# Korinin38/raytracing-hw

Hardware: AMD Instinct MI355X
Metric: Mrays/sec + frame time, Sponza 1920x1080x256spp at 1/2/4/8 MI355X (higher is better)
Workload: dtype f32

## Files before the change

### raytracing-hw_amd/csrc/rt_device.hip

```cpp
#include <hip/hip_runtime.h>
#include <hipcub/hipcub.hpp>

#include <algorithm>
#include <chrono>
#include <cstdio>
#include <cstdlib>
#include <cstring>
#include <mutex>
#include <string>
#include <thread>
#include <vector>

#include "rt_path.h"
#include "rt_wavefront.h"
#include <type_traits>
#include "rt_mega.h"
#include "rt_quant_lut.h"
#include "rt_scene.h"
#include "rt_bvh_layout.h"
#include "rt_launch_plan.h"
#include "rt_select.h"
#include "rt_frame_plan.h"
#include "rt_gbuffer.h"
#include "rt_denoise.h"

using rtd::Counters;
using rtd::DevScene;
using rtd::ShardGeom;
using rtd::shard_row;

#ifndef RT_MEGA_WPE
#define RT_MEGA_WPE 5
#endif
constexpr int kMegaWpe = RT_MEGA_WPE;
#ifndef RT_SPEC_WPE
#define RT_SPEC_WPE 4
#endif
constexpr int kMegaWpeSpec = RT_SPEC_WPE;
#ifndef RT_SHADE_MIN
#define RT_SHADE_MIN 48
#endif
#ifndef RT_SPEC_SHADE_MIN
#define RT_SPEC_SHADE_MIN 44
#endif
constexpr int kSpecShadeMin = RT_SPEC_SHADE_MIN;
constexpr int kShadeMin = RT_SHADE_MIN;
#ifndef RT_PACK_TRAV
#define RT_PACK_TRAV 1
#endif
constexpr bool kPackTrav = RT_PACK_TRAV != 0;
#ifndef RT_INV_RECOMPUTE
#define RT_INV_RECOMPUTE 1
#endif
constexpr bool kInvRecompute = RT_INV_RECOMPUTE != 0;
#ifndef RT_COOP_LEAVES
#define RT_COOP_LEAVES 8
#endif
constexpr int kCoopLeavesPlain = RT_COOP_LEAVES;
#ifndef RT_SPEC_COOP_LEAVES
#define RT_SPEC_COOP_LEAVES 12
#endif
constexpr int kCoopLeavesSpec = RT_SPEC_COOP_LEAVES;
#ifndef RT_SPEC_MASK_LOAD
#define RT_SPEC_MASK_LOAD 1
#endif
constexpr bool kSpecMaskLoad = RT_SPEC_MASK_LOAD != 0;
#ifndef RT_PLAIN_FAR_DIST2
#define RT_PLAIN_FAR_DIST2 RT_FAR_DIST2
#endif
#ifndef RT_SPEC_FAR_DIST2
#define RT_SPEC_FAR_DIST2 0
#endif
constexpr bool kPlainFarDist2 = RT_PLAIN_FAR_DIST2 != 0, kSpecFarDist2 = RT_SPEC_FAR_DIST2 != 0;
#ifndef RT_COOP_ROUND_MIN
#define RT_COOP_ROUND_MIN 8
#endif
constexpr int kCoopRoundMinPlain = RT_COOP_ROUND_MIN;
#ifndef RT_ORDER_SPP
#define RT_ORDER_SPP 1
#endif
#ifndef RT_ORDER_RADIUS
#define RT_ORDER_RADIUS 4
#endif
constexpr int kOrderSpp = RT_ORDER_SPP;
constexpr int kOrderRadius = RT_ORDER_RADIUS;
using rtp::kClaimStride;
constexpr int kWfRefill = 8;
constexpr unsigned kWfChunk = 64;
constexpr double kWfCompactBelow = 0.75;

struct rt_device_blob {
    std::vector<uint8_t> bytes;
    size_t o_tri, o_attr, o_tan, o_node, o_light, o_lnode, o_mf, o_mt, o_nt, o_ti, o_tx, o_lut;
};

struct rt_device_scene {
    int device = -1;
    void *buf = nullptr;
    DevScene ds{};
    unsigned long long *counters = nullptr;
    unsigned long long *queue = nullptr;
    int cu_count = 0;
    void *wf_buf = nullptr;
    long long wf_cap = 0;
    int wf_D = 0;
    rtd::WfState wf{};
    float4 *wf_queue[2] = {nullptr, nullptr};
    float4 *wf_hits = nullptr;
    unsigned *wf_count = nullptr;
    unsigned *wf_fetch = nullptr;
    unsigned *wf_host_count = nullptr;
    float *fast_part = nullptr;
    size_t fast_part_bytes = 0;
    void *order_buf = nullptr;
    size_t order_bytes = 0;
    struct Frame {
        hipStream_t stream = nullptr, cp_stream = nullptr;
        void *buf[2] = {nullptr, nullptr};
        size_t bytes[2] = {0, 0};
        hipEvent_t copied[2] = {nullptr, nullptr};
        hipEvent_t finished = nullptr;
        hipEvent_t last = nullptr;
        void *root_buf = nullptr;
        size_t root_bytes = 0;
    } fr;
};

#define HIP_TRY(expr)                                                                          \
    do {                                                                                       \
        hipError_t _e = (expr);                                                                \
        if (_e != hipSuccess)                                                                  \
            return rt_fail(RT_ERR_DEVICE, std::string(#expr) + ": " + hipGetErrorString(_e)); \
    } while (0)

namespace {

struct DeviceGuard {
    int prev = -1;
    bool ok = false;
    explicit DeviceGuard(int dev) {
        if (hipGetDevice(&prev) != hipSuccess) prev = -1;
        ok = hipSetDevice(dev) == hipSuccess;
    }
    ~DeviceGuard() {
        if (prev >= 0) (void)hipSetDevice(prev);
    }
};

struct EventSet {
    std::vector<hipEvent_t> ev;
    hipError_t make(hipEvent_t &e) {
        hipError_t r = hipEventCreate(&e);
        if (r == hipSuccess) ev.push_back(e);
        return r;
    }
    ~EventSet() {
        for (hipEvent_t e : ev) (void)hipEventDestroy(e);
    }
};

hipError_t grow(void **p, size_t *cap, size_t need) {
    if (*p && *cap >= need) return hipSuccess;
    if (*p) (void)hipFree(*p);
    *p = nullptr;
    *cap = 0;
    hipError_t e = hipMalloc(p, need ? need : 256);
    if (e == hipSuccess) *cap = need;
    return e;
}

}

__constant__ uint32_t k_quant_thr[256];
__global__ void __launch_bounds__(256) rt_finish_kernel(const float *sum, long long n, float normalizer,
                                                         uint8_t *rgb) {
    __shared__ float thr[256];
    thr[threadIdx.x] = __uint_as_float(k_quant_thr[threadIdx.x]);
    __syncthreads();
    for (long long i = (long long)blockIdx.x * blockDim.x + threadIdx.x; i < n; i += (long long)gridDim.x * blockDim.x) {
        float x = sum[i];
        x *= normalizer;
        const float num = x * (x * 2.51f + 0.03f);
        const float den = x * (x * 2.43f + 0.59f) + 0.14f;
        const float v = rtv::smax(rtv::smin(num / den, 1.f), 0.f);
        int q = 0;
        if (!isnan(v)) {
            int lo = 0;
#pragma unroll
            for (int step = 128; step > 0; step >>= 1)
                if (lo + step <= 255 && thr[lo + step] <= v) lo += step;
            q = lo;
        }
        rgb[i] = (uint8_t)q;
    }
}

__global__ void __launch_bounds__(256) rt_finish_counts_kernel(const float *sum, const int32_t *counts, long long n,
                                                                uint8_t *rgb) {
    __shared__ float thr[256];
    thr[threadIdx.x] = __uint_as_float(k_quant_thr[threadIdx.x]);
    __syncthreads();
    for (long long i = (long long)blockIdx.x * blockDim.x + threadIdx.x; i < n; i += (long long)gridDim.x * blockDim.x) {
        const int32_t c = counts[i / 3];
        float x = sum[i];
        x *= rtsel::count_normalizer(c);
        const float num = x * (x * 2.51f + 0.03f);
        const float den = x * (x * 2.43f + 0.59f) + 0.14f;
        const float v = rtv::smax(rtv::smin(num / den, 1.f), 0.f);
        int q = 0;
        if (c > 0 && !isnan(v)) {
            int lo = 0;
#pragma unroll
            for (int step = 128; step > 0; step >>= 1)
                if (lo + step <= 255 && thr[lo + step] <= v) lo += step;
            q = lo;
        }
        rgb[i] = (uint8_t)q;
    }
}

#ifdef RT_MEGA_PROF
#include "rt_mega_prof.h"
#endif
template <bool COUNT, bool FAST = false, bool LSPLIT = false, bool SPEC = false, bool CHAIN = false>
__global__ void __launch_bounds__(256) __attribute__((amdgpu_waves_per_eu(SPEC ? kMegaWpeSpec : kMegaWpe, 8)))
rt_mega_kernel(DevScene sc_in, ShardGeom g, rtd::WfState st, int spp, float *out, unsigned long long *counters,
               unsigned long long *queue, const int *order, unsigned *cost, int cs, int mode) {
    constexpr bool kSpec = SPEC && !COUNT && !FAST && !LSPLIT;
    constexpr bool kChain = CHAIN && !COUNT && !FAST && !LSPLIT;
    constexpr bool kFastChain = CHAIN && FAST && !COUNT && !LSPLIT && !SPEC;
    const int park_below = kFastChain ? 0 : rtp::mode_park_below(mode), resume_pct = kFastChain ? 0 : rtp::mode_resume_pct(mode);
    const uint4 *resume = kSpec && resume_pct > 0 ? (const uint4 *)queue[rtd::kQueueParkList] : nullptr;
    const long long n_items = kFastChain ? st.n * (long long)mode
                              : FAST     ? g.n_pixels * (long long)((spp + cs - 1) / cs)
                                         : (kChain || (kSpec && resume)) ? st.n : g.n_pixels;
    const int lane = threadIdx.x & 63;
    __shared__ float lut[256];
    for (int k = threadIdx.x; k < 256; k += blockDim.x) lut[k] = sc_in.lut[k];
    __syncthreads();
    DevScene sc = sc_in;
    sc.lut = lut;
    Counters cnt{0, 0, 0, 0, 0, 0, 0};
    constexpr int kK = kSpec ? rtd::kLdsStackSpec : rtd::kLdsStack;
    uint2 spill[rtd::kStack - kK];
    rtd::LdsStackT<kK> S{spill};
    const rtd::GlobalNodes nodes{sc.node};
    const rtd::NodeRec root = rtd::load_node(sc.node, 0);
    std::conditional_t<kSpec, rtd::MegaLane, rtd::MegaLaneU> L;
    L.pix = -1;
    L.state = rtd::M_IDLE;
    L.T.phase = rtd::TP_POP;
    L.T.sp = 0;
#if defined(RT_DEBUG_CHECKS)
    if (rt_debug_poison) {
        L.T.phase = 0x7ffffffd;
        L.T.sp = 0x3ffffff;
    }
#endif
    L.wbase = (uint32_t)__builtin_amdgcn_readfirstlane((int)threadIdx.x) & ~63u;
    bool exhausted = false;
    bool tail = false, wave_room = false;
#ifdef RT_MEGA_PROF
    unsigned long long pf[7] = {0, 0, 0, 0, 0, 0, 0};
    if (threadIdx.x < 8) rt_prof_lds[threadIdx.x] = 0;
    if (threadIdx.x < 16) rtd::spec_prof_lds[threadIdx.x] = 0;
    if ((threadIdx.x & 63) == 0) rtd::spec_wave_t0_lds[threadIdx.x >> 6] = wall_clock64();
    __syncthreads();
    long long tp = clock64();
    const unsigned long long wt0 = wall_clock64();
    TbAcc tbk;
#endif
    rtd::SpecClaim claim{queue + rtd::kQueueResume, 0, n_items, resume, 0, false,
                         resume ? (const int *)queue[rtd::kQueueResumeMap] : nullptr};
    bool park = false;
    if constexpr (kSpec) {
        if (resume) {
            const long long waves = (long long)gridDim.x * (blockDim.x >> 6);
            const long long dealt = (n_items * resume_pct + 99) / 100;
            const int per = (int)std::min<long long>(64, std::max<long long>(1, (dealt + waves - 1) / waves));
            const long long p = (rtd::mega_slot() >> 6) * per + lane;
            bool xk = false;
            rtd::Rng xs{0u, 0u, 0.f};
            if (lane < per && p < n_items) {
                const rtd::Parked q = rtd::parked_item(resume, claim.ridx, p);
                if (q.pix != rtd::kNoPark) {
                    rtd::mega_resume(L, sc, g, q, root);
                    xk = true;
                    xs = q.x;
                }
            }
            exhausted = true;
            claim.base = waves * per;
            claim.keep = per;
            claim.open = claim.base < n_items;
            if (lane == 0) rtd::spec_hint_take();
            rtd::spec_convert(L, sc, g, rtd::SpecView{(uint4 *)st.mid, st.lanes, rtd::mega_slot() - lane}, lane, xk, xs);
            tail = true;
#ifdef RT_MEGA_PROF
            if (lane == 0) RT_SPEC_STAT(7, 1);
#endif
        }
    }
#if defined(RT_DEBUG_CHECKS)
    unsigned long long dbg_iter = 0;
#endif
    for (;;) {
#if defined(RT_DEBUG_CHECKS)
        if (++dbg_iter > (1ull << 22)) {
            const unsigned long long w = (unsigned long long)__popcll(__ballot(L.state == rtd::M_TRAV)) |
                                         (unsigned long long)__popcll(__ballot(L.state == rtd::M_READY)) << 8 |
                                         (unsigned long long)__popcll(__ballot(L.state == rtd::M_DONE)) << 16 |
                                         (unsigned long long)__popcll(__ballot(L.state == rtd::M_DONE_NEW)) << 24 |
                                         (unsigned long long)__popcll(__ballot(L.state == rtd::M_IDLE)) << 32 |
                                         (unsigned long long)tail << 40 | (unsigned long long)park << 41 |
                                         (unsigned long long)exhausted << 42 | (unsigned long long)wave_room << 43;
            RT_CHECK(false, 15, w, (void)0);
            if constexpr (kSpec) {
                const rtd::SpecView V{(uint4 *)st.mid, st.lanes, rtd::mega_slot() - lane};
                const uint4 a = *V.w(0, lane), b = *V.w(1, lane), c = *V.w(2, lane), d = *V.w(3, lane), j = *V.w(4, lane);
                if (atomicAdd(&rt_debug_prints, 1u) < 64u)
                    printf("[stuck] blk %d lane %d state %d pix %d s %d | job tag %u | rec pix %u f %u n %u e %u meta %u tab %08x%08x\n",
                           (int)blockIdx.x, lane, L.state, L.pix, rtd::lane_ctr(L).s, j.x, a.x, a.y, a.z, a.w, b.w, d.w, c.w);
            }
            break;
        }
#endif
        if (!kSpec && !COUNT && !FAST && park) {
            if (L.state == rtd::M_IDLE && L.pix >= 0) {
                rtd::park_pixel((uint4 *)queue[rtd::kQueueParkList], rtd::mega_slot_of(L), L.pix, rtd::lane_ctr(L).s, rtd::lane_rng(L),
                                rtd::lane_sum(L));
                L.pix = -1;
            }
        }
        if (!exhausted) {
            const bool need = L.pix < 0 && (kClaimStride == 1 || lane % kClaimStride == 0);
            const unsigned long long m = __ballot(need);
            if (m) {
                const int leader = __ffsll((unsigned long long)m) - 1;
                const unsigned cm = (unsigned)__popcll(m);
                const int below = (int)__builtin_amdgcn_mbcnt_hi((uint32_t)(m >> 32), __builtin_amdgcn_mbcnt_lo((uint32_t)m, 0u));
                unsigned long long base = 0;
                if (need && below == 0) base = atomicAdd(queue + rtd::kQueueRender, (unsigned long long)cm);
                base = __shfl(base, leader, 64);
                if (need) {
                    const long long p = (long long)base + below;
                    if (p < n_items) {
                        if constexpr (kFastChain)
                            rtd::mega_assign_fast_chain<COUNT>(L, sc, g, p, st.n, order, cs, spp, root, cnt, rtd::chain_of(queue));
                        else if (FAST) rtd::mega_assign_fast<COUNT>(L, sc, g, p, cs, spp, root, cnt);
                        else if constexpr (kChain)
                            rtd::mega_assign_chain<COUNT>(L, sc, g, order ? order[p] : (int)p, root, cnt, rtd::chain_of(queue), spp);
                        else rtd::mega_assign<COUNT>(L, sc, g, order ? order[p] : (int)p, root, cnt);
                    }
                }
                if ((long long)base + cm >= n_items) exhausted = true;
            }
        }
        if constexpr (kSpec) {
            if (exhausted && !tail) {
                if (lane == 0) rtd::spec_hint_take();
                if constexpr (kChain)
                    rtd::spec_convert_chain(L, sc, g, rtd::SpecView{(uint4 *)st.mid, st.lanes, rtd::mega_slot() - lane}, lane,
                                            rtd::chain_of(queue));
                else
                    rtd::spec_convert(L, sc, g, rtd::SpecView{(uint4 *)st.mid, st.lanes, rtd::mega_slot() - lane}, lane);
                tail = true;
                wave_room = false;
#ifdef RT_MEGA_PROF
                if (lane == 0) RT_SPEC_STAT(7, 1);
#endif
            }
            if (tail) {
                wave_room |= rtd::spec_hint_take();
                if (__any(L.state == rtd::M_DONE_NEW) || (wave_room && __any(L.state == rtd::M_IDLE))) {
#ifdef RT_MEGA_PROF
                    const long long c0 = clock64();
                    tbk.c[5] += 1;
#endif
                    wave_room = rtd::spec_manage<kChain>(rtd::SpecLanes{L}, sc, g,
                                                 rtd::SpecView{(uint4 *)st.mid, st.lanes, rtd::mega_slot() - lane}, spp,
                                                 out, root, claim);
#ifdef RT_MEGA_PROF
                    if (lane == 0) {
                        RT_SPEC_STAT(0, 1);
                        RT_SPEC_STAT(1, clock64() - c0);
                    }
#endif
                }
                if (!__any(L.state != rtd::M_IDLE)) break;
            } else if (!__any(L.pix >= 0)) {
                break;
            }
        } else if constexpr (kFastChain) {
            if (!__any(L.pix >= 0)) {
                if (exhausted) break;
                continue;
            }
        } else if (!__any(L.pix >= 0)) {
            break;
        }
        if (!kSpec && park_below > 0 && exhausted && !park) park = rtp::park_rule(__popcll(__ballot(L.pix >= 0)), park_below);
        const int nr = __popcll(__ballot(L.state == rtd::M_READY || (LSPLIT && L.state == rtd::M_LREADY)));
        const int nt = __popcll(__ballot(L.state == rtd::M_TRAV || (LSPLIT && L.state == rtd::M_LTRAV)));
        const bool shade_now = nr > 0 && (nr >= (kSpec ? kSpecShadeMin : kShadeMin) || nt == 0);
        if constexpr (kSpec) {
            if (shade_now) __builtin_amdgcn_s_setprio(0);
            else __builtin_amdgcn_s_setprio(1);
        }
#ifdef RT_MEGA_PROF
        {
            const long long t1 = clock64();
            pf[2] += (unsigned long long)(t1 - tp);
            tp = t1;
            pf[shade_now ? 3 : 4] += 1;
            pf[shade_now ? 5 : 6] += (unsigned long long)(shade_now ? nr : nt);
            tbk.at(wt0);
            if (shade_now) {
                tbk.c[3] += 1;
                tbk.c[4] += (unsigned long long)nr;
            }
        }
#endif
        if (!LSPLIT && !shade_now) {
            int kt = nt;
            int leaf_defer = 0;
            do {
                if (rtd::trav_step_coop<COUNT, kSpec ? kCoopLeavesSpec : kCoopLeavesPlain, kSpec && kSpecMaskLoad,
                                        kSpec ? rtd::kLeafDefer : (COUNT ? 0 : rtd::kLeafDeferPlain),
                                        kSpec ? kSpecFarDist2 : kPlainFarDist2>(
                        sc, L.r, L.T, S, nodes, cnt, L.state == rtd::M_TRAV, kSpec ? st.round_min : kCoopRoundMinPlain,
                        rtd::NoHook{}, &leaf_defer))
                    L.state = rtd::M_READY;
                const unsigned long long rb = __ballot(L.state == rtd::M_READY), tb = __ballot(L.state == rtd::M_TRAV);
                kt = __popcll(tb);
                if (kt == 0 || __popcll(rb) >= (kSpec ? kSpecShadeMin : kShadeMin)) break;
#ifdef RT_MEGA_PROF
                pf[4] += 1;
                pf[6] += (unsigned long long)kt;
                tbk.c[0] += 1;
                tbk.c[1] += (unsigned long long)kt;
                tbk.c[2] += (unsigned long long)__popcll(__ballot(L.state != rtd::M_IDLE));
#endif
            } while (true);
        } else if (kPackTrav && !LSPLIT && !kSpec && !FAST) {
            RT_CHECK((unsigned)L.T.phase < 4u && (unsigned)L.state < 8u && (unsigned)L.T.sp <= (unsigned)rtd::kStack, 14,
                     (unsigned)L.T.phase | (unsigned long long)(unsigned)L.state << 32, (void)0);
            uint32_t pk = ((uint32_t)L.T.phase & 3u) | ((uint32_t)L.state & 7u) << 2 | ((uint32_t)L.T.sp & 127u) << 5;
            asm volatile("" : "+v"(pk));
            if (L.state == rtd::M_READY) {
                L.T.phase = 0;
                L.T.sp = 0;
                rtd::mega_shade<COUNT, FAST, kChain>(L, sc, g, st, spp, out, cost, root, S, cnt, kSpec && tail, park, queue);
            } else {
                L.T.phase = (int)(pk & 3u);
                L.state = (int)((pk >> 2) & 7u);
                L.T.sp = (int)(pk >> 5);
            }
        } else {
            rtd::mega_iterate<COUNT, decltype(S), decltype(nodes), FAST, LSPLIT, kChain>(L, shade_now, sc, g, st, spp, out,
                                                                                       cost, root, S, nodes, cnt,
                                                                                       kSpec && tail, false, queue);
            if (kInvRecompute && shade_now) L.r.inv = rtv::divv(rtd::V3{1.f, 1.f, 1.f}, L.r.d);
        }
        if (kPackTrav && kInvRecompute && !LSPLIT && !kSpec && !FAST && shade_now)
            L.r.inv = rtv::divv(rtd::V3{1.f, 1.f, 1.f}, L.r.d);

#ifdef RT_MEGA_PROF
        {
            const long long t1 = clock64();
            pf[shade_now ? 0 : 1] += (unsigned long long)(t1 - tp);
            tp = t1;
        }
#endif
    }
#ifdef RT_MEGA_PROF
    tbk.flush(tbk.b);
    if (lane == 0) {
        for (int k = 0; k < 7; ++k) atomicAdd(&g_mega_prof[k], pf[k]);
        atomicAdd(&g_mega_prof[7], 1ull);
        const unsigned wi = atomicAdd(&g_wave_n, 1u);
        if (wi < (unsigned)kProfWaves) {
            g_wave_t[2 * wi] = wt0;
            g_wave_t[2 * wi + 1] = wall_clock64();
        }
    }
    __syncthreads();
    if (threadIdx.x < 8) atomicAdd(&g_mega_seg[threadIdx.x], rt_prof_lds[threadIdx.x]);
    if (threadIdx.x < 16) atomicAdd(&rtd::g_spec_prof[threadIdx.x], rtd::spec_prof_lds[threadIdx.x]);
#endif
    rtd::counters_flush<COUNT>(cnt, counters);
}

__global__ void __launch_bounds__(256) rt_fast_reduce_kernel(const float *__restrict__ part, float *__restrict__ out,
                                                             long long n3, int chunks) {
    const long long i = (long long)blockIdx.x * blockDim.x + threadIdx.x;
    if (i >= n3) return;
    float s = 0.f;
    for (int c = 0; c < chunks; ++c) s += part[(long long)c * n3 + i];
    out[i] = s;
}

struct FastPartials {
    const float *part;
    long long n_list, i;
    RT_HD float operator()(int k, int ch) const { return part[3 * ((long long)k * n_list + i) + ch]; }
};
__global__ void __launch_bounds__(256) rt_fast_fold_chain_kernel(uint4 *chain, const int *items, long long n_list, int units,
                                                                  int c, int target, const float *__restrict__ part,
                                                                  float *sums) {
    const long long i = (long long)blockIdx.x * blockDim.x + threadIdx.x;
    if (i >= n_list) return;
    const long long p = items ? (long long)items[i] : i;
    rtd::FastRec q = rtd::fast_rec(chain, p);
    const int own = rtfu::units_of(q.r.next, target, c);
    if (own < 1 || own > units) return;
    rtfu::fold(q.r, target, c, FastPartials{part, n_list, i});
    rtd::fast_rec_store(chain, p, q.r);
    float s[3];
    rtfu::reported(q.r, c, s);
    sums[3 * p + 0] = s[0];
    sums[3 * p + 1] = s[1];
    sums[3 * p + 2] = s[2];
}

__global__ void __launch_bounds__(256) rt_order_iota_kernel(int *ids, long long n) {
    const long long i = (long long)blockIdx.x * blockDim.x + threadIdx.x;
    if (i < n) ids[i] = (int)i;
}

__global__ void __launch_bounds__(256) rt_order_box_kernel(const unsigned *in, unsigned *out, long long n, int width,
                                                           int r, int dir) {
    const long long p = (long long)blockIdx.x * blockDim.x + threadIdx.x;
    if (p >= n) return;
    const long long rows = n / width, k = p / width, i = p % width;
    unsigned s = 0;
    for (int d = -r; d <= r; ++d) {
        const long long kk = dir ? k + d : k, ii = dir ? i : i + d;
        if (kk >= 0 && kk < rows && ii >= 0 && ii < width) s += in[kk * width + ii];
    }
    out[p] = s;
}

__global__ void __launch_bounds__(256) rt_order_spread_kernel(const int *sorted, int *order, long long n,
                                                              long long groups, long long per) {
    const long long q = (long long)blockIdx.x * blockDim.x + threadIdx.x;
    if (q >= n) return;
    const long long m = n < groups * per ? n : groups * per;
    long long r = q;
    if (q < m) {
        const long long gi = q / per, j = q % per, a = m / per, b = m % per;
        r = j * a + (j < b ? j : b) + gi;
    }
    order[q] = sorted[r];
}

__global__ void __launch_bounds__(256) rt_park_keys_kernel(const uint4 *park, long long n, int spp, const unsigned *est,
                                                           unsigned *keys, int *ids) {
    const long long i = (long long)blockIdx.x * blockDim.x + threadIdx.x;
    if (i >= n) return;
    const rtd::Parked q = rtd::parked(park, i);
    unsigned long long k = 0;
    if (q.pix != rtd::kNoPark) k = (unsigned long long)(spp - (int)q.s) * ((unsigned long long)est[q.pix] + 1ull);
    keys[i] = k > 0xffffffffull ? 0xffffffffu : (unsigned)k;
    ids[i] = (int)i;
}
__global__ void rt_set_u64_kernel(unsigned long long *dst, unsigned long long v) { *dst = v; }

__global__ void __launch_bounds__(256) wf_init_kernel(DevScene sc, ShardGeom g, rtd::WfState st, long long n,
                                                       float4 *qout, unsigned *cout) {
    for (long long base = (long long)blockIdx.x * blockDim.x; base < n; base += (long long)gridDim.x * blockDim.x) {
        const long long i = base + threadIdx.x;
        const bool valid = i < n;
        if (valid) rtd::store_qray(sc, qout, (unsigned)i, (int)i, rtd::wf_init_slot(sc, g, st, i));
        rtd::queue_slot(valid, cout);
    }
}

template <bool COUNT>
__global__ void __launch_bounds__(256) wf_extend_kernel(DevScene sc, const float4 *qin, const unsigned *count,
                                                         unsigned npos, float4 *hits, unsigned *fetch,
                                                         unsigned *next_count, unsigned long long *counters) {
    const unsigned n = npos ? npos : *count;
    if (blockIdx.x == 0 && threadIdx.x == 0) {
        atomicAdd(&counters[7], (unsigned long long)n);
        *next_count = 0;
    }
    Counters cnt{0, 0, 0, 0, 0, 0, 0};
    uint2 spill[rtd::kStack - rtd::kLdsStackWf];
    rtd::LdsStackT<rtd::kLdsStackWf> S{spill};
    const int lane = threadIdx.x & 63;
    const rtd::GlobalNodes nodes{sc.node};
    const rtd::NodeRec root = rtd::load_node(sc.node, 0);
    unsigned q = 0, lo = 0, hi = 0;
    bool busy = false, exhausted = false;
    rtd::Ray r;
    rtd::TravState T;
    for (;;) {
        const unsigned long long m = __ballot(!busy);
        const unsigned idle = (unsigned)__popcll(m);
        if (!exhausted && (idle >= (unsigned)kWfRefill || idle == 64)) {
            const unsigned rank = (unsigned)__popcll(m & ((1ull << lane) - 1ull));
            unsigned got = 0, mine = 0xffffffffu;
            while (got < idle) {
                if (lo >= hi) {
                    unsigned b = 0;
                    if (lane == 0) b = atomicAdd(fetch, kWfChunk);
                    b = __shfl(b, 0, 64);
                    if (b >= n) {
                        exhausted = true;
                        break;
                    }
                    lo = b;
                    hi = b + kWfChunk < n ? b + kWfChunk : n;
                }
                const unsigned k = hi - lo < idle - got ? hi - lo : idle - got;
                if (!busy && rank >= got && rank < got + k) mine = lo + (rank - got);
                lo += k;
                got += k;
            }
            if (mine != 0xffffffffu) {
                q = mine;
                uint32_t bits;
                int slot;
                r = rtd::load_qray_trav(qin, q, bits, slot);
                if (slot >= 0) {
                    busy = rtd::trav_start<COUNT>(bits, root.a, root.b, T, cnt);
                    if (!busy) rtd::store_hit(hits, q, T.best);
                }
            }
        }
        if (busy && rtd::trav_step<COUNT>(sc, r, T, S, nodes, cnt)) {
            rtd::store_hit(hits, q, T.best);
            busy = false;
        }
        if (exhausted && !__any(busy)) break;
    }
    rtd::counters_flush<COUNT>(cnt, counters);
}

constexpr int kMatLds = 64;
struct ShadeLds {
    float lut[512];
    float mf[kMatLds * 12];
    int mt[kMatLds * 4];
    double nt[kMatLds * 16];
};

template <bool COUNT, bool MAT_LDS>
__global__ void __launch_bounds__(256) wf_shade_kernel(DevScene sc_in, ShardGeom g, rtd::WfState st, int spp,
                                                        const float4 *qin, const unsigned *cin, unsigned npos,
                                                        const float4 *hits, float4 *qout, unsigned *cout,
                                                        int dense_out, unsigned *fetch, float *out,
                                                        unsigned long long *counters) {
    __shared__ ShadeLds L;
    for (int k = threadIdx.x; k < 512; k += blockDim.x) L.lut[k] = sc_in.lut[k];
    if (MAT_LDS) {
        for (int k = threadIdx.x; k < sc_in.n_meshes * 12; k += blockDim.x) L.mf[k] = sc_in.mesh_f[k];
        for (int k = threadIdx.x; k < sc_in.n_meshes * 4; k += blockDim.x) L.mt[k] = sc_in.mesh_tex[k];
        for (int k = threadIdx.x; k < sc_in.n_meshes * 16; k += blockDim.x) L.nt[k] = sc_in.mesh_nt[k];
    }
    __syncthreads();
    DevScene sc = sc_in;
    sc.lut = L.lut;
    if (MAT_LDS) {
        sc.mesh_f = L.mf;
        sc.mesh_tex = L.mt;
        sc.mesh_nt = L.nt;
    }
    const unsigned n = npos ? npos : *cin;
    if (blockIdx.x == 0 && threadIdx.x == 0) *fetch = 0;
    Counters cnt{0, 0, 0, 0, 0, 0, 0};
    for (unsigned base = blockIdx.x * blockDim.x; base < n; base += gridDim.x * blockDim.x) {
        const unsigned q = base + threadIdx.x;
        int slot = -1;
        bool next = false;
        rtd::Ray r;
        if (q < n) {
            r = rtd::load_qray(qin, q, slot);
            if (slot >= 0) {
                const rtd::Hit h = rtd::load_hit(hits, q);
                next = rtd::wf_shade_slot<COUNT>(sc, g, st, spp, slot, r, h, out, cnt);
            }
        }
        const unsigned p = rtd::queue_slot(next, cout);
        if (dense_out) {
            if (next) rtd::store_qray(sc, qout, q, slot, r);
            else if (q < n) rtd::store_qray_inactive(qout, q);
        } else if (next) {
            rtd::store_qray(sc, qout, p, slot, r);
        }
    }
    rtd::counters_flush<COUNT>(cnt, counters);
}

__global__ void __launch_bounds__(256) rt_rays_kernel(DevScene sc, long long n, const float *org, const float *dir,
                                                       float *out_f, long long *out_i) {
    const long long k = (long long)blockIdx.x * blockDim.x + threadIdx.x;
    if (k >= n) return;
    rtd::Ray r = rtd::make_ray(rtv::V3{org[3 * k], org[3 * k + 1], org[3 * k + 2]},
                               rtv::V3{dir[3 * k], dir[3 * k + 1], dir[3 * k + 2]});
    Counters c1{0, 0, 0, 0, 0, 0, 0}, c2{0, 0, 0, 0, 0, 0, 0};
    rtd::Hit h;
    const bool ok = rtd::closest_hit<true>(sc, r, h, c1);
    const float lp = sc.n_lights ? rtd::light_pdf<true>(sc, r.o, r.d, c2) : 0.f;
    out_f[4 * k + 0] = ok ? h.t : 0.f;
    out_f[4 * k + 1] = ok ? h.u : 0.f;
    out_f[4 * k + 2] = ok ? h.v : 0.f;
    out_f[4 * k + 3] = lp;
    out_i[6 * k + 0] = ok;
    out_i[6 * k + 1] = ok ? h.prim : -1;
    out_i[6 * k + 2] = c1.aabb;
    out_i[6 * k + 3] = c1.tri;
    out_i[6 * k + 4] = c2.laabb;
    out_i[6 * k + 5] = c2.ltri;
}

namespace {

template <class T>
size_t append(std::vector<uint8_t> &blob, const std::vector<T> &v, size_t pre = 0) {
    size_t off = rtp::align_up(blob.size()) + pre;
    blob.resize(off + v.size() * sizeof(T));
    if (!v.empty()) std::memcpy(blob.data() + off, v.data(), v.size() * sizeof(T));
    return off;
}

void tile_textures(const std::vector<uint32_t> &info, const std::vector<uint8_t> &texels, std::vector<uint32_t> &info_out,
                   std::vector<uint32_t> &out) {
    const size_t n = info.size() / 4;
    info_out = info;
    out.clear();
    for (size_t t = 0; t < n; ++t) {
        const uint32_t off = info[4 * t], w = info[4 * t + 1], h = info[4 * t + 2];
        const uint32_t tw = (w + 3) / 4, th = (h + 3) / 4;
        const size_t base = out.size();
        info_out[4 * t] = (uint32_t)base;
        out.resize(base + (size_t)tw * th * 16, 0u);
        for (uint32_t y = 0; y < h; ++y)
            for (uint32_t x = 0; x < w; ++x) {
                uint32_t v;
                std::memcpy(&v, &texels[4 * ((size_t)off + (size_t)y * w + x)], 4);
                out[base + ((size_t)(y >> 2) * tw + (x >> 2)) * 16 + (y & 3) * 4 + (x & 3)] = v;
            }
    }
}

int ensure_blob(rt_scene *s) {
    if (s->blob) return RT_OK;
    if (s->bvh_depth + 2 >= (uint32_t)rtd::kStack || s->light_bvh_depth + 2 >= (uint32_t)rtd::kStack)
        return rt_fail(RT_ERR_LIMIT, "BVH deeper than the device traversal stack (" + std::to_string(rtd::kStack) + ")");
    if (s->ray_depth > rtd::kMaxDepth) return rt_fail(RT_ERR_LIMIT, "ray_depth exceeds device limit");
    for (size_t k = 0; k < s->node.size() / 8; ++k) {
        uint32_t a, b;
        std::memcpy(&a, &s->node[8 * k + 6], 4);
        std::memcpy(&b, &s->node[8 * k + 7], 4);
        if (a >= rtd::kFrameMaxA || b >= 1024u)
            return rt_fail(RT_ERR_LIMIT, "scene too large for the device BVH frame packing (2^22 nodes/triangles, 255 per leaf)");
    }
    auto *b = new rt_device_blob();
    std::vector<uint8_t> &blob = b->bytes;
    b->o_tri = append(blob, s->tri);
    b->o_attr = append(blob, s->tri_attr);
    b->o_tan = append(blob, s->tri_tan);
    b->o_node = append(blob, rtd::bfs_nodes(s->node), 32);
    b->o_light = append(blob, s->light);
    b->o_lnode = append(blob, s->light_node);
    b->o_mf = append(blob, s->mesh_f);
    b->o_mt = append(blob, s->mesh_tex);
    b->o_nt = append(blob, s->mesh_nt);
    std::vector<uint32_t> tinfo, tiled;
    tile_textures(s->tex_info, s->texels, tinfo, tiled);
    b->o_ti = append(blob, tinfo);
    b->o_tx = append(blob, tiled);
    std::vector<float> lut(512);
    rtd::fill_decode_lut(lut.data());
    b->o_lut = append(blob, lut);
    blob.resize(rtp::align_up(blob.size()) + 256);
    s->blob = b;
    return RT_OK;
}

void free_device_scene(rt_device_scene *d) {
    if (!d) return;
    DeviceGuard guard(d->device);
    if (guard.ok) {
        for (hipStream_t q : {d->fr.stream, d->fr.cp_stream})
            if (q) (void)hipStreamSynchronize(q);
        for (void *p : {d->buf, (void *)d->counters, (void *)d->queue, d->wf_buf, (void *)d->wf_count,
                        (void *)d->wf_fetch, (void *)d->fast_part, d->order_buf, d->fr.buf[0], d->fr.buf[1], d->fr.root_buf})
            if (p) (void)hipFree(p);
        if (d->wf_host_count) (void)hipHostFree(d->wf_host_count);
        for (hipEvent_t e : {d->fr.copied[0], d->fr.copied[1], d->fr.finished, d->fr.last})
            if (e) (void)hipEventDestroy(e);
        for (hipStream_t q : {d->fr.stream, d->fr.cp_stream})
            if (q) (void)hipStreamDestroy(q);
    }
    delete d;
}

hipError_t ensure_frame_streams(rt_device_scene *d) {
    hipError_t e = hipSuccess;
    if (!d->fr.stream) e = hipStreamCreateWithFlags(&d->fr.stream, hipStreamNonBlocking);
    if (e == hipSuccess && !d->fr.cp_stream) e = hipStreamCreateWithFlags(&d->fr.cp_stream, hipStreamNonBlocking);
    for (hipEvent_t *ev : {&d->fr.copied[0], &d->fr.copied[1], &d->fr.finished, &d->fr.last})
        if (e == hipSuccess && !*ev) e = hipEventCreateWithFlags(ev, hipEventDisableTiming);
    return e;
}

int ensure_device_scene(rt_scene *s, int device) {
    if (device < 0 || device >= kRtMaxDevices) return rt_fail(RT_ERR_DEVICE, "no HIP device " + std::to_string(device));
    if (s->dev[device]) return RT_OK;
    int ndev = 0;
    HIP_TRY(hipGetDeviceCount(&ndev));
    if (device >= ndev) return rt_fail(RT_ERR_DEVICE, "no HIP device " + std::to_string(device));
    int rc = ensure_blob(s);
    if (rc) return rc;
    const rt_device_blob &b = *s->blob;
    DeviceGuard guard(device);
    if (!guard.ok) return rt_fail(RT_ERR_DEVICE, "hipSetDevice(" + std::to_string(device) + ") failed");
    rt_device_scene *d = new rt_device_scene();
    d->device = device;
    hipError_t e = hipMalloc(&d->buf, b.bytes.size());
    if (e == hipSuccess) e = hipMemcpy(d->buf, b.bytes.data(), b.bytes.size(), hipMemcpyHostToDevice);
    if (e == hipSuccess) e = hipMalloc((void **)&d->counters, rtd::kCounterWords * sizeof(unsigned long long));
    if (e == hipSuccess) e = hipMalloc((void **)&d->queue, rtd::kQueueWords * sizeof(unsigned long long));
    hipDeviceProp_t prop;
    if (e == hipSuccess) e = hipGetDeviceProperties(&prop, device);
    if (e != hipSuccess) {
        free_device_scene(d);
        return rt_fail(RT_ERR_DEVICE, std::string("scene upload: ") + hipGetErrorString(e));
    }
    d->cu_count = prop.multiProcessorCount;
    uint8_t *base = (uint8_t *)d->buf;
    DevScene &ds = d->ds;
    ds.tri = (const float4 *)(base + b.o_tri);
    ds.tri_attr = (const float4 *)(base + b.o_attr);
    ds.tri_tan = (const float4 *)(base + b.o_tan);
    ds.node = (const float4 *)(base + b.o_node);
    ds.light = (const float4 *)(base + b.o_light);
    ds.light_node = (const float4 *)(base + b.o_lnode);
    ds.mesh_f = (const float *)(base + b.o_mf);
    ds.mesh_tex = (const int *)(base + b.o_mt);
    ds.mesh_nt = (const double *)(base + b.o_nt);
    ds.tex_info = (const uint4 *)(base + b.o_ti);
    ds.texels = (const uint32_t *)(base + b.o_tx);
    ds.lut = (const float *)(base + b.o_lut);
    ds.n_lights = (int)(s->light.size() / 16);
    ds.n_tris = (int)(s->tri.size() / 12);
    ds.n_nodes = (int)(s->node.size() / 8);
    ds.n_meshes = (int)(s->mesh_f.size() / 12);
    ds.ray_depth = s->ray_depth;
    ds.max_distance = s->max_distance;
    ds.width = s->width;
    ds.height = s->height;
    ds.fwidth = (float)s->width;
    ds.fheight = (float)s->height;
    std::memcpy(ds.cam_pos, s->cam_pos, sizeof ds.cam_pos);
    std::memcpy(ds.cam_axes, s->cam_axes, sizeof ds.cam_axes);
    std::memcpy(ds.tan_fov, s->tan_half_fov, sizeof ds.tan_fov);
    s->dev[device] = d;
    return RT_OK;
}

int ensure_wf(rt_device_scene *d, long long n, int D) {
    if (d->wf_buf && d->wf_cap >= n && d->wf_D == D) return RT_OK;
    if (d->wf_buf) (void)hipFree(d->wf_buf);
    d->wf_buf = nullptr;
    d->wf_cap = 0;
    const long long cap = ((n + 255) / 256) * 256;
    const int planes = 8 + 9 * D + 20
                       + 2 * 4 * rtd::kQRec + 4;
    const size_t bytes = (size_t)cap * 4 * (size_t)planes;
    HIP_TRY(hipMalloc(&d->wf_buf, bytes));
    if (!d->wf_count) HIP_TRY(hipMalloc((void **)&d->wf_count, 16));
    if (!d->wf_fetch) HIP_TRY(hipMalloc((void **)&d->wf_fetch, 16));
    if (!d->wf_host_count) HIP_TRY(hipHostMalloc((void **)&d->wf_host_count, 16, hipHostMallocDefault));
    float *f = (float *)d->wf_buf;
    auto take = [&](long long k) { float *p = f; f += (size_t)cap * k; return p; };
    rtd::WfState &w = d->wf;
    w.n = n;
    w.D = D;
    d->wf_queue[0] = (float4 *)take(4 * rtd::kQRec);
    d->wf_queue[1] = (float4 *)take(4 * rtd::kQRec);
    d->wf_hits = (float4 *)take(4);
    w.st = (float4 *)take(8);
    w.rec_ab = (float4 *)take(8 * D);
    w.rec_c = take(D);
    w.mid = (float4 *)take(20);
    {
        const unsigned long long park = (unsigned long long)(uintptr_t)d->wf_queue[0];
        HIP_TRY(hipMemcpy(d->queue + rtd::kQueueParkList, &park, sizeof park, hipMemcpyHostToDevice));
    }
    d->wf_cap = cap;
    d->wf_D = D;
    return RT_OK;
}

template <class K>
long long resident_blocks(rt_device_scene *d, K kernel) {
    int per_cu = 0;
    if (hipOccupancyMaxActiveBlocksPerMultiprocessor(&per_cu, kernel, 256, 0) != hipSuccess || per_cu < 1) per_cu = 1;
    return (long long)d->cu_count * per_cu;
}
template <class K>
unsigned persistent_blocks(rt_device_scene *d, K kernel, long long work) {
    const long long need = (work + 255) / 256;
    const long long b = std::min<long long>(need, resident_blocks(d, kernel));
    return (unsigned)std::max<long long>(b, 1);
}

struct LaunchTimer {
    bool on = false;
    std::vector<hipEvent_t> ev[2];
    hipError_t mark(int k, hipStream_t s) {
        if (!on) return hipSuccess;
        hipEvent_t e;
        hipError_t r = hipEventCreate(&e);
        if (r != hipSuccess) return r;
        ev[k].push_back(e);
        return hipEventRecord(e, s);
    }
    hipError_t collect(double ms[2], uint64_t n[2]) {
        hipError_t r = hipSuccess;
        for (int k = 0; k < 2; ++k) {
            ms[k] = 0.0;
            n[k] = ev[k].size() / 2;
            for (size_t j = 0; j + 1 < ev[k].size(); j += 2) {
                float t = 0.f;
                if (r == hipSuccess) r = hipEventElapsedTime(&t, ev[k][j], ev[k][j + 1]);
                ms[k] += t;
            }
            for (hipEvent_t e : ev[k]) (void)hipEventDestroy(e);
            ev[k].clear();
        }
        return r;
    }
    ~LaunchTimer() {
        for (auto &v : ev)
            for (hipEvent_t e : v) (void)hipEventDestroy(e);
    }
};

int launch_wavefront(rt_device_scene *d, const ShardGeom &g, int spp, int depth, float *d_out, hipStream_t stream,
                     bool count, LaunchTimer &timer) {
    if (depth < 1 || depth > 15) return rt_fail(RT_ERR_LIMIT, "wavefront path: ray_depth must be in [1, 15]");
    if (spp >= (1 << 20)) return rt_fail(RT_ERR_LIMIT, "wavefront path: spp must be < 2^20");
    if (g.n_pixels >= (1LL << 31)) return rt_fail(RT_ERR_LIMIT, "wavefront path: shards below 2^31 pixels");
    int rc = ensure_wf(d, g.n_pixels, depth);
    if (rc) return rc;
    rtd::WfState w = d->wf;
    w.n = g.n_pixels;
    const long long n = g.n_pixels;
    HIP_TRY(hipMemsetAsync(d->wf_count, 0, 16, stream));
    HIP_TRY(hipMemsetAsync(d->wf_fetch, 0, 16, stream));
    auto extend = count ? wf_extend_kernel<true> : wf_extend_kernel<false>;
    const unsigned ext_blocks = persistent_blocks(d, extend, n);
    const bool mat_lds = d->ds.n_meshes <= kMatLds;
    auto shade = count ? (mat_lds ? wf_shade_kernel<true, true> : wf_shade_kernel<true, false>)
                       : (mat_lds ? wf_shade_kernel<false, true> : wf_shade_kernel<false, false>);
    const unsigned sh_blocks = persistent_blocks(d, shade, n);
    const unsigned init_blocks = (unsigned)std::min<long long>((n + 255) / 256, (long long)d->cu_count * 8);
    hipLaunchKernelGGL(wf_init_kernel, dim3(init_blocks), dim3(256), 0, stream, d->ds, g, w, n, d->wf_queue[0],
                       &d->wf_count[0]);
    HIP_TRY(hipGetLastError());
    bool dense = true, to_compact = false;
    const long long max_iter = (long long)spp * depth + 16;
    int cur = 0;
    for (long long it = 0;; ++it) {
        if (it > max_iter) return rt_fail(RT_ERR_DEVICE, "wavefront path did not drain (internal error)");
        float4 *qi = d->wf_queue[cur], *qo = d->wf_queue[1 - cur];
        const unsigned npos = dense ? (unsigned)n : 0u;
        HIP_TRY(timer.mark(0, stream));
        hipLaunchKernelGGL(extend, dim3(ext_blocks), dim3(256), 0, stream, d->ds, qi, &d->wf_count[cur], npos,
                           d->wf_hits, d->wf_fetch, &d->wf_count[1 - cur], d->counters);
        HIP_TRY(timer.mark(0, stream));
        HIP_TRY(timer.mark(1, stream));
        const int dense_out = dense && !to_compact;
        hipLaunchKernelGGL(shade, dim3(sh_blocks), dim3(256), 0, stream, d->ds, g, w, spp, qi, &d->wf_count[cur], npos,
                           d->wf_hits, qo, &d->wf_count[1 - cur], dense_out, d->wf_fetch, d_out, d->counters);
        if (to_compact) dense = false;
        HIP_TRY(timer.mark(1, stream));
        HIP_TRY(hipGetLastError());
        cur = 1 - cur;
        if ((it & 7) == 7) {
            HIP_TRY(hipMemcpyAsync(d->wf_host_count, &d->wf_count[cur], 4, hipMemcpyDeviceToHost, stream));
            HIP_TRY(hipStreamSynchronize(stream));
            if (d->wf_host_count[0] == 0) break;
            if (dense && (double)d->wf_host_count[0] < kWfCompactBelow * (double)n) to_compact = true;
        }
    }
    return RT_OK;
}

using MegaKernel = void (*)(DevScene, ShardGeom, rtd::WfState, int, float *, unsigned long long *, unsigned long long *,
                            const int *, unsigned *, int, int);
MegaKernel mega_kernel_of(const rtp::Variant &v);

struct OrderBuf {
    unsigned *cost, *cost_sorted;
    int *ids, *sorted, *order;
    void *tmp;
    unsigned *park_keys, *park_keys_sorted;
    int *resume_map;
    static size_t array_bytes(long long n) { return rtp::align_up((size_t)n * 4); }
    static size_t bytes(long long n, size_t tmp_bytes) { return 5 * array_bytes(n) + tmp_bytes; }
    OrderBuf(void *base, long long n_pixels) {
        uint8_t *b = (uint8_t *)base;
        const size_t arr = array_bytes(n_pixels);
        cost = (unsigned *)b;
        cost_sorted = park_keys = (unsigned *)(b + arr);
        ids = (int *)(b + 2 * arr);
        sorted = (int *)(b + 3 * arr);
        order = (int *)(b + 4 * arr);
// ... 1462 lines not shown
            HIP_TRY(hipStreamWaitEvent(q, s->dev[d]->fr.last, 0));
        } else {
            DeviceGuard gp(d);
            if (!gp.ok) return rt_fail(RT_ERR_DEVICE, "hipSetDevice failed");
            HIP_TRY(hipEventSynchronize(s->dev[d]->fr.last));
        }
    }
    hipLaunchKernelGGL(rt_rows_scatter_kernel, dim3(4, (unsigned)H), dim3(256), 0, q, (const uint8_t *)(buf + f.o_stage_u8),
                       frame_u8, row_map, H, (long long)f.row_u8);
    HIP_TRY(hipGetLastError());
    if (out_sum) {
        hipLaunchKernelGGL(rt_rows_scatter_kernel, dim3(8, (unsigned)H), dim3(256), 0, q,
                           (const uint8_t *)(buf + f.o_stage_f), frame_f, row_map, H, (long long)f.row_f);
        HIP_TRY(hipGetLastError());
    }
    if (out_rgb) HIP_TRY(hipMemcpyAsync(out_rgb, frame_u8, (size_t)H * f.row_u8, hipMemcpyDeviceToHost, q));
    if (out_sum) HIP_TRY(hipMemcpyAsync(out_sum, frame_f, (size_t)H * f.row_f, hipMemcpyDeviceToHost, q));
    HIP_TRY(hipStreamSynchronize(q));
    return RT_OK;
}

}

extern "C" {

int rt_render_frame(rt_scene *s, const rt_params *p, int32_t n_shards, const int32_t *devices, uint8_t *out_rgb,
                    float *out_sum, rt_stats *st) {
    if (!s || !p || (!out_rgb && !out_sum)) return rt_fail(RT_ERR_ARG, "rt_render_frame: NULL argument");
    if (int rc = check_flags(p, "rt_render_frame")) return rc;
    if (const rtp::Refusal r = rtp::frame_check_devices(n_shards, devices)) return rt_fail(r.code, r.msg);
    int ndev = 0;
    HIP_TRY(hipGetDeviceCount(&ndev));
    const rtp::FrameIn in{s->width, s->height, n_shards, devices, norm_row_block(p), p->spp > 0 ? p->spp : s->samples,
                          ndev, out_sum != nullptr};
    if (const rtp::Refusal r = rtp::frame_check(in)) return rt_fail(r.code, r.msg);
    if (int rc = ensure_blob(s)) return rc;
    const rtp::FramePlan f = rtp::plan_frame(in);
    if (f.refused) return rt_fail(f.refused.code, f.refused.msg);
    if (int rc = frame_prepare_devices(s, f)) return rc;
    if (int rc = frame_setup_root(s, f)) return rc;
    const size_t nu = f.uniq.size();
    FrameRun run{s, p, f, (uint8_t *)s->dev[f.root()]->fr.root_buf, std::vector<rt_stats>(f.n),
                 std::vector<int>(nu, RT_OK), std::vector<std::string>(nu)};
    std::vector<std::thread> threads;
    for (size_t ui = 1; ui < nu; ++ui) threads.emplace_back(&FrameRun::work, &run, ui);
    run.work(0);
    for (std::thread &t : threads) t.join();
    const auto t0 = std::chrono::steady_clock::now();
    for (size_t ui = 0; ui < nu; ++ui)
        if (run.rcs[ui] != RT_OK) {
            for (int d : f.uniq) {
                DeviceGuard g(d);
                (void)hipStreamSynchronize(s->dev[d]->fr.cp_stream);
            }
            return rt_fail(run.rcs[ui], "device " + std::to_string(f.uniq[ui]) + ": " + run.errs[ui]);
        }
    if (int rc = frame_assemble(s, f, out_rgb, out_sum)) return rc;
    const double gather_ms = std::chrono::duration<double, std::milli>(std::chrono::steady_clock::now() - t0).count();
    if (st) rtp::merge_frame_stats(f, run.stats.data(), gather_ms, st);
    return RT_OK;
}

int rt_render_multi(rt_scene *s, const rt_params *p, int32_t n_devices, float *out, rt_stats *st) {
    if (!s || !p || !out) return rt_fail(RT_ERR_ARG, "rt_render_multi: NULL argument");
    if (int rc = check_flags(p, "rt_render_multi")) return rc;
    int ndev = 0;
    HIP_TRY(hipGetDeviceCount(&ndev));
    const int n = n_devices > 0 ? n_devices : ndev;
    if (n < 1 || n > ndev || n > kRtMaxDevices)
        return rt_fail(RT_ERR_DEVICE, "rt_render_multi: " + std::to_string(n) + " devices requested, " +
                                          std::to_string(ndev) + " visible");
    return rt_render_frame(s, p, n, nullptr, nullptr, out, st);
}

int rt_intersect_rays(rt_scene *s, int64_t n, const float *org, const float *dir, float *out_f, int64_t *out_i) {
    if (!s || n < 0 || (n > 0 && (!org || !dir || !out_f || !out_i))) return rt_fail(RT_ERR_ARG, "rt_intersect_rays: bad argument");
    if (n == 0) return RT_OK;
    int rc = ensure_device_scene(s, 0);
    if (rc) return rc;
    DeviceGuard guard(0);
    if (!guard.ok) return rt_fail(RT_ERR_DEVICE, "hipSetDevice failed");
    float *d_o = nullptr, *d_d = nullptr, *d_f = nullptr;
    long long *d_i = nullptr;
    const size_t v3 = (size_t)n * 3 * sizeof(float);
    hipError_t e = hipMalloc(&d_o, v3);
    if (e == hipSuccess) e = hipMalloc(&d_d, v3);
    if (e == hipSuccess) e = hipMalloc(&d_f, (size_t)n * 4 * sizeof(float));
    if (e == hipSuccess) e = hipMalloc(&d_i, (size_t)n * 6 * sizeof(long long));
    if (e == hipSuccess) e = hipMemcpy(d_o, org, v3, hipMemcpyHostToDevice);
    if (e == hipSuccess) e = hipMemcpy(d_d, dir, v3, hipMemcpyHostToDevice);
    if (e == hipSuccess) {
        hipLaunchKernelGGL(rt_rays_kernel, dim3((unsigned)((n + 255) / 256)), dim3(256), 0, nullptr, s->dev[0]->ds,
                           (long long)n, d_o, d_d, d_f, d_i);
        e = hipGetLastError();
    }
    if (e == hipSuccess) e = hipMemcpy(out_f, d_f, (size_t)n * 4 * sizeof(float), hipMemcpyDeviceToHost);
    if (e == hipSuccess) e = hipMemcpy(out_i, d_i, (size_t)n * 6 * sizeof(long long), hipMemcpyDeviceToHost);
    (void)hipFree(d_o);
    (void)hipFree(d_d);
    (void)hipFree(d_f);
    (void)hipFree(d_i);
    if (e != hipSuccess) return rt_fail(RT_ERR_DEVICE, std::string("rt_intersect_rays: ") + hipGetErrorString(e));
    return RT_OK;
}

#if defined(RT_DEBUG_CHECKS)
int rt_debug_take(unsigned long long *word) {
    unsigned long long z = 0;
    HIP_TRY(hipDeviceSynchronize());
    HIP_TRY(hipMemcpyFromSymbol(word, HIP_SYMBOL(rt_debug_word), sizeof z));
    HIP_TRY(hipMemcpyToSymbol(HIP_SYMBOL(rt_debug_word), &z, sizeof z));
    return RT_OK;
}
int rt_debug_set_poison(int on) {
    HIP_TRY(hipMemcpyToSymbol(HIP_SYMBOL(rt_debug_poison), &on, sizeof on));
    return RT_OK;
}
#endif

__global__ void __launch_bounds__(256) rcp_check_kernel(unsigned long long *bad) {
    unsigned long long local = 0;
    for (uint64_t i = (uint64_t)blockIdx.x * blockDim.x + threadIdx.x; i < (1ull << 32);
         i += (uint64_t)gridDim.x * blockDim.x) {
        const float x = __uint_as_float((uint32_t)i);
        const float ax = fabsf(x);
        if (!(ax >= 0x1p-126f && ax < 0x1p125f)) continue;
        const float a = rtd::rcp_ieee(x), b = 1.f / x;
        local += __float_as_uint(a) != __float_as_uint(b);
    }
    for (int off = 32; off > 0; off >>= 1) local += __shfl_down(local, off, 64);
    if ((threadIdx.x & 63) == 0 && local) atomicAdd(bad, local);
}

__global__ void __launch_bounds__(256) decode_check_kernel(unsigned long long *bad) {
    unsigned long long local = 0;
    if (blockIdx.x == 0) {
        const uint32_t b = threadIdx.x;
        local += __float_as_uint(rtd::unorm8(b)) != __float_as_uint((float)b / 255.f);
    }
    for (uint64_t i = (uint64_t)blockIdx.x * blockDim.x + threadIdx.x; i < 2147483647ull;
         i += (uint64_t)gridDim.x * blockDim.x) {
        const uint32_t x = (uint32_t)i;
#pragma unroll
        for (uint32_t f = 0; f < 2; ++f) {
            uint32_t ux, uf;
            rtd::rng_word_unpack(rtd::rng_word_pack(x, f), ux, uf);
            local += (ux != x) | (uf != f);
        }
    }
    for (int off = 32; off > 0; off >>= 1) local += __shfl_down(local, off, 64);
    if ((threadIdx.x & 63) == 0 && local) atomicAdd(bad, local);
}

__global__ void __launch_bounds__(256) far_check_kernel(unsigned long long *bad) {
    const uint32_t i = blockIdx.x * blockDim.x + threadIdx.x;
    unsigned long long local = 0;
    {
        const uint32_t j = i / (uint32_t)rtd::kFarCaseXs, v = i % (uint32_t)rtd::kFarCaseXs;
        const float acc = rtd::far_case_acc(j % (uint32_t)rtd::kFarCaseExps, j / (uint32_t)rtd::kFarCaseExps);
        const float x = rtd::far_case_x(acc, (int)v);
        local += rtd::far_gt(x, acc) != (sqrtf(x) > acc);
    }
    if (i < 54u) {
        const float accs[6] = {0.f, -0.f, 1e-45f, 0x1p-126f, 1.f, 1e9f};
        const float xs[9] = {0.f, 1e-45f, 0x1p-126f, 1.f, 4.f, 9.f, 1e18f, __builtin_inff(), __builtin_nanf("")};
        const float acc = accs[i / 9u], x = xs[i % 9u];
        local += rtd::far_gt(x, acc) != (sqrtf(x) > acc);
    }
    if (i < 132u) {
        const float x = i < 129u ? rtd::far_case_step(rtd::kFarMax2, (int)i - 64)
                                 : (i == 129u ? 0.f : (i == 130u ? __builtin_inff() : __builtin_nanf("")));
        local += (x > rtd::kFarMax2) != (sqrtf(x) > 1e9f);
    }
    for (int off = 32; off > 0; off >>= 1) local += __shfl_down(local, off, 64);
    if ((threadIdx.x & 63) == 0 && local) atomicAdd(bad, local);
}

}

template <int kLeaves>
__global__ void __launch_bounds__(256) coop_check_kernel(const float4 *tri, int n_tris, const float4 *nodes,
                                                          const float4 *rays, const uint2 *leaves, int n_cases,
                                                          int round_min, unsigned long long *bad) {
    const int i = (int)(blockIdx.x * blockDim.x + threadIdx.x);
    const bool valid = i < n_cases;
    DevScene sc{};
    sc.tri = tri;
    sc.n_tris = n_tris;
    sc.node = nodes;
    sc.n_nodes = 2;
    const float4 ro = rays[2 * (valid ? i : 0)], rdv = rays[2 * (valid ? i : 0) + 1];
    const rtd::Ray r = rtd::make_ray(rtv::V3{ro.x, ro.y, ro.z}, rtv::V3{rdv.x, rdv.y, rdv.z});
    const uint2 lf = leaves[valid ? i : 0];
    rtd::TravState T;
    T.best.t = 1e9f;
    T.best.u = T.best.v = 0.f;
    T.best.prim = -1;
    T.acc = 1e9f;
    T.sp = 0;
    T.a = T.b = 0;
    T.k = lf.x;
    T.kend = lf.y;
    T.phase = rtd::TP_LEAF;
    Counters cnt{0, 0, 0, 0, 0, 0, 0};
    uint2 spill[rtd::kStack - 4];
    rtd::LdsStackT<4> S{spill};
    const rtd::GlobalNodes gn{nodes};
    bool active = valid;
    for (int it = 0; it < 64 && __any(active); ++it)
        if (rtd::trav_step_coop<false, kLeaves, false>(sc, r, T, S, gn, cnt, active, round_min)) active = false;
    if (rtd::kUvRecompute && valid && T.best.prim >= 0) rtd::hit_uv(sc, r, T.best);
    float acc = 1e9f;
    rtd::Hit best{1e9f, 0.f, 0.f, -1};
    for (uint32_t k = lf.x; valid && k < lf.y; ++k) {
        const float4 q0 = tri[3 * k], q1 = tri[3 * k + 1], q2 = tri[3 * k + 2];
        rtd::TriHit h;
        if (rtd::tri_hit_bl(rtv::V3{q0.x, q0.y, q0.z}, rtv::V3{q0.w, q1.x, q1.y}, rtv::V3{q1.z, q1.w, q2.x}, r, h)) {
            acc = h.t < acc ? h.t : acc;
            if (h.t < best.t) best = rtd::Hit{h.t, h.u, h.v, (int)k};
        }
    }
    unsigned long long local = 0;
    if (valid)
        local = (active | (T.best.prim != best.prim) | (__float_as_uint(T.best.t) != __float_as_uint(best.t)) |
                 (__float_as_uint(T.best.u) != __float_as_uint(best.u)) |
                 (__float_as_uint(T.best.v) != __float_as_uint(best.v)) | (__float_as_uint(T.acc) != __float_as_uint(acc)))
                    ? 1ull : 0ull;
    for (int off = 32; off > 0; off >>= 1) local += __shfl_down(local, off, 64);
    if ((threadIdx.x & 63) == 0 && local) atomicAdd(bad, local);
}

namespace {
void coop_cases(std::vector<float> &tri, std::vector<float> &rays, std::vector<uint32_t> &leaves, int n_cases) {
    uint64_t x = 0x9e3779b97f4a7c15ull;
    auto rnd = [&]() {
        x ^= x << 13; x ^= x >> 7; x ^= x << 17;
        return (float)((x >> 40) & 0xffffff) / 16777216.f;
    };
    const int groups = 512;
    tri.assign((size_t)groups * 8 * 12, 0.f);
    std::vector<float> cen((size_t)groups * 3);
    for (int gi = 0; gi < groups; ++gi) {
        float v0[3], U[3], V[3];
        for (int c = 0; c < 3; ++c) {
            v0[c] = rnd() * 4.f - 2.f;
            U[c] = rnd() * 2.f - 1.f;
            V[c] = rnd() * 2.f - 1.f;
            cen[3 * gi + c] = v0[c] + (U[c] + V[c]) / 3.f;
        }
        for (int t = 0; t < 8; ++t) {
            float *o = &tri[((size_t)gi * 8 + t) * 12];
            float a[3], u[3], w[3];
            for (int c = 0; c < 3; ++c) {
                a[c] = v0[c]; u[c] = U[c]; w[c] = V[c];
                if (t == 2 || t == 3) { a[c] = v0[c] + 0.25f * U[c]; }
                if (t == 5) { a[c] = rnd() * 4.f - 2.f; u[c] = rnd() * 2.f - 1.f; w[c] = rnd() * 2.f - 1.f; }
            }
            if (t == 4) a[1] = __builtin_nanf("");
            if (t == 7) u[0] = __builtin_inff();
            for (int c = 0; c < 3; ++c) { o[c] = a[c]; o[3 + c] = u[c]; o[6 + c] = w[c]; }
        }
    }
    rays.assign((size_t)n_cases * 8, 0.f);
    leaves.assign((size_t)n_cases * 2, 0u);
    for (int i = 0; i < n_cases; ++i) {
        const int gi = (int)(rnd() * groups) % groups;
        float o[3], d[3];
        for (int c = 0; c < 3; ++c) {
            o[c] = rnd() * 20.f - 10.f;
            d[c] = cen[3 * gi + c] + (rnd() - 0.5f) * 0.2f - o[c];
        }
        for (int c = 0; c < 3; ++c) { rays[8 * (size_t)i + c] = o[c]; rays[8 * (size_t)i + 4 + c] = d[c]; }
        const uint32_t len = 1u + (uint32_t)(rnd() * 7.f) % 7u, first = (uint32_t)gi * 8u + (uint32_t)(rnd() * 8.f) % 8u;
        const uint32_t k0 = std::min<uint32_t>(first, (uint32_t)groups * 8u - len);
        leaves[2 * (size_t)i] = k0;
        leaves[2 * (size_t)i + 1] = k0 + len;
    }
}
}

extern "C" {

int rt_device_selfcheck(int32_t which, uint64_t *mismatches) {
    if (!mismatches) return rt_fail(RT_ERR_ARG, "rt_device_selfcheck: null output");
    if (which < 0 || which > 3) return rt_fail(RT_ERR_ARG, "rt_device_selfcheck: unknown check " + std::to_string(which));
    unsigned long long *d = nullptr;
    HIP_TRY(hipMalloc((void **)&d, sizeof *d));
    hipError_t e = hipMemset(d, 0, sizeof *d);
    void *cbuf = nullptr;
    if (e == hipSuccess) {
        if (which == 0) {
            hipLaunchKernelGGL(rcp_check_kernel, dim3(4096), dim3(256), 0, nullptr, d);
        } else if (which == 1) {
            hipLaunchKernelGGL(decode_check_kernel, dim3(4096), dim3(256), 0, nullptr, d);
        } else if (which == 3) {
            hipLaunchKernelGGL(far_check_kernel, dim3((1u << 24) / 256u), dim3(256), 0, nullptr, d);
        } else {
            const int n_cases = 1 << 16;
            std::vector<float> tri, rays;
            std::vector<uint32_t> leaves;
            coop_cases(tri, rays, leaves, n_cases);
            const size_t bt = tri.size() * 4 + 64, br = rays.size() * 4, bl = leaves.size() * 4, bn = 256;
            e = hipMalloc(&cbuf, bt + br + bl + bn);
            uint8_t *b = (uint8_t *)cbuf;
            if (e == hipSuccess) e = hipMemset(cbuf, 0, bt + br + bl + bn);
            if (e == hipSuccess) e = hipMemcpy(b, tri.data(), tri.size() * 4, hipMemcpyHostToDevice);
            if (e == hipSuccess) e = hipMemcpy(b + bt, rays.data(), br, hipMemcpyHostToDevice);
            if (e == hipSuccess) e = hipMemcpy(b + bt + br, leaves.data(), bl, hipMemcpyHostToDevice);
            const int n_tris = (int)(tri.size() / 12);
            const unsigned blocks = (unsigned)(n_cases / 256);
            if (e == hipSuccess) {
                for (int rm : {65, 1}) {
                    hipLaunchKernelGGL(coop_check_kernel<8>, dim3(blocks), dim3(256), 0, nullptr, (const float4 *)b,
                                       n_tris, (const float4 *)(b + bt + br + bl), (const float4 *)(b + bt),
                                       (const uint2 *)(b + bt + br), n_cases, rm, d);
                    hipLaunchKernelGGL(coop_check_kernel<16>, dim3(blocks), dim3(256), 0, nullptr, (const float4 *)b,
                                       n_tris, (const float4 *)(b + bt + br + bl), (const float4 *)(b + bt),
                                       (const uint2 *)(b + bt + br), n_cases, rm, d);
                }
            }
        }
        if (e == hipSuccess) e = hipGetLastError();
    }
    unsigned long long h = 0;
    if (e == hipSuccess) e = hipMemcpy(&h, d, sizeof h, hipMemcpyDeviceToHost);
    (void)hipFree(d);
    if (cbuf) (void)hipFree(cbuf);
    if (e != hipSuccess) return rt_fail(RT_ERR_DEVICE, std::string("rt_device_selfcheck: ") + hipGetErrorString(e));
    *mismatches = h;
    return RT_OK;
}

int32_t rt_device_count(void) {
    int n = 0;
    if (hipGetDeviceCount(&n) != hipSuccess) return 0;
    return n;
}

int rt_device_synchronize(void) {
    HIP_TRY(hipDeviceSynchronize());
    return RT_OK;
}

}
```

### raytracing-hw_amd/csrc/rt_mega.h

```cpp
#pragma once
#include "rt_fast_units.h"
#include "rt_wavefront.h"
#if !defined(__HIPCC__)
#include <algorithm>
#endif

namespace rtd {

#if defined(__HIPCC__)
__device__ __forceinline__ long long mega_slot() { return (long long)blockIdx.x * blockDim.x + threadIdx.x; }
#else
inline thread_local long long g_mega_slot = 0;
inline long long mega_slot() { return g_mega_slot; }
#endif

__device__ __forceinline__ const float4 *mega_nodes(const DevScene &sc) { return sc.node; }

enum MegaState : int { M_IDLE = 0, M_TRAV = 1, M_READY = 2, M_LTRAV = 3, M_LREADY = 4, M_DONE_NEW = 5, M_DONE = 6 };
static_assert(M_DONE < 8, "rt_mega_kernel packs a lane's state in 3 bits (RT_PACK_TRAV)");

template <class TS>
struct MegaLaneT {
    int pix;
    uint32_t ctr;
// ... 141 lines not shown
    const uint32_t seed = (uint32_t)(py * sc.width + px) % 2147483647u;
    return Rng{seed == 0 ? 1u : seed, 0u, 0.f};
}

template <bool COUNT, class ML>
__device__ __forceinline__ void mega_assign(ML &L, const DevScene &sc, const ShardGeom &g, int p,
                                            const NodeRec &root, Counters &cnt) {
    L.pix = p;
    lane_ctr_set(L, LaneCtr{0, 0, 0});
    lane_sum_set(L, V3{0.f, 0.f, 0.f});
    L.work0 = cnt.aabb + cnt.tri + cnt.laabb + cnt.ltri;
    lane_rng_set(L, pixel_seed(sc, g, p));
    mega_sample<COUNT>(L, sc, g, root, cnt);
}

template <class ML>
__device__ __forceinline__ void mega_resume(ML &L, const DevScene &sc, const ShardGeom &g, const Parked &q,
                                            const NodeRec &root) {
    L.pix = (int)q.pix;
    lane_ctr_set(L, LaneCtr{(int)q.s, 0, 0});
    lane_sum_set(L, q.sum);
    lane_rng_set(L, q.x);
    Counters cnt{0, 0, 0, 0, 0, 0, 0};
    mega_sample<false>(L, sc, g, root, cnt);
}

template <bool COUNT, class ML>
__device__ __forceinline__ void mega_assign_fast(ML &L, const DevScene &sc, const ShardGeom &g, long long q,
                                                 int cs, int spp, const NodeRec &root, Counters &cnt) {
    const long long c = q / g.n_pixels;
    const int p = (int)(q - c * g.n_pixels);
    L.pix = p;
    L.dst = q;
    const int s0 = (int)c * cs;
    lane_ctr_set(L, LaneCtr{s0, 0, 0});
    L.send = s0 + cs < spp ? s0 + cs : spp;
    lane_sum_set(L, V3{0.f, 0.f, 0.f});
    L.work0 = cnt.aabb + cnt.tri + cnt.laabb + cnt.ltri;
    int px, py;
    shard_xy(g, p, px, py);
    L.gpix = (uint32_t)(py * sc.width + px);
    mega_sample<COUNT, true>(L, sc, g, root, cnt);
}

constexpr uint32_t kNoPark = 0xffffffffu;
__device__ __forceinline__ void park_pixel(uint4 *park, long long slot, int pix, int s, const Rng &r, V3 sum) {
    park[2 * slot] = make_uint4((uint32_t)pix, (uint32_t)s, rng_word_pack(r.x, r.saved_avail), __float_as_uint(r.saved));
    park[2 * slot + 1] = make_uint4(__float_as_uint(sum.x), __float_as_uint(sum.y), __float_as_uint(sum.z), 0u);
}

enum QueueWord : int {
    kQueueRender = 0,
    kQueueOrder = 1,
    kQueueParkCount = 2,
    kQueueResume = 3,
    kQueueParkList = 4,
    kQueueResumeMap = 5,
    kChainWord = 16,
    kQueueWords = 32,
};
constexpr int kOrderCounters = 8, kCounterWords = 16;
__device__ __forceinline__ uint4 *chain_of(const unsigned long long *queue) { return (uint4 *)queue[kChainWord]; }
__device__ __forceinline__ void chain_store(uint4 *chain, uint32_t pix, uint32_t s, const Rng &r, V3 sum) {
    park_pixel(chain, (long long)pix, (int)pix, (int)s, r, sum);
}
__device__ __forceinline__ void chain_init(uint4 *chain, const DevScene &sc, const ShardGeom &g, int p) {
    chain_store(chain, (uint32_t)p, 0u, pixel_seed(sc, g, p), V3{0.f, 0.f, 0.f});
}
template <bool COUNT, class ML>
__device__ __forceinline__ void mega_assign_chain(ML &L, const DevScene &sc, const ShardGeom &g, int p,
                                                  const NodeRec &root, Counters &cnt, const uint4 *chain,
                                                  int spp = 0x7fffffff) {
    const Parked q = parked(chain, p);
    RT_CHECK((int)q.s < spp, 16, p, (void)0);
    L.pix = p;
    lane_ctr_set(L, LaneCtr{(int)q.s, 0, 0});
    lane_sum_set(L, q.sum);
    L.work0 = cnt.aabb + cnt.tri + cnt.laabb + cnt.ltri;
    lane_rng_set(L, q.x);
    mega_sample<COUNT>(L, sc, g, root, cnt);
}
struct FastRec {
    uint32_t pix;
    rtfu::Rec r;
};
__device__ __forceinline__ FastRec fast_rec(const uint4 *chain, long long p) {
    const uint4 a = chain[2 * p], b = chain[2 * p + 1];
    FastRec q;
    q.pix = a.x;
    q.r.next = (int)a.y;
    q.r.total[0] = __uint_as_float(a.z);
    q.r.total[1] = __uint_as_float(a.w);
    q.r.total[2] = __uint_as_float(b.x);
    q.r.open[0] = __uint_as_float(b.y);
    q.r.open[1] = __uint_as_float(b.z);
    q.r.open[2] = __uint_as_float(b.w);
    return q;
}
__device__ __forceinline__ void fast_rec_store(uint4 *chain, long long p, const rtfu::Rec &r) {
    chain[2 * p] = make_uint4((uint32_t)p, (uint32_t)r.next, __float_as_uint(r.total[0]), __float_as_uint(r.total[1]));
    chain[2 * p + 1] = make_uint4(__float_as_uint(r.total[2]), __float_as_uint(r.open[0]), __float_as_uint(r.open[1]),
                                  __float_as_uint(r.open[2]));
}
template <bool COUNT, class ML>
__device__ __forceinline__ bool mega_assign_fast_chain(ML &L, const DevScene &sc, const ShardGeom &g, long long q,
                                                       long long n_list, const int *order, int cs, int spp,
                                                       const NodeRec &root, Counters &cnt, const uint4 *chain) {
    const int k = (int)(q / n_list);
    const long long i = q - (long long)k * n_list;
    const int p = order ? order[i] : (int)i;
    RT_CHECK(p >= 0 && p < g.n_pixels, 17, p, return false);
    const FastRec rec = fast_rec(chain, p);
    const rtfu::Range u = rtfu::unit_range(rec.r.next, spp, cs, k);
    RT_CHECK((u.s0 < u.s1) == (k < rtfu::units_of(rec.r.next, spp, cs)), 17, q, return false);
    if (u.s0 >= u.s1) return false;
    L.pix = p;
    L.dst = q;
    lane_ctr_set(L, LaneCtr{u.s0, 0, 0});
    L.send = u.s1;
    const bool cont = rtfu::unit_continues(rec.r.next, cs, k);
    lane_sum_set(L, cont ? V3{rec.r.open[0], rec.r.open[1], rec.r.open[2]} : V3{0.f, 0.f, 0.f});
    L.work0 = cnt.aabb + cnt.tri + cnt.laabb + cnt.ltri;
    int px, py;
    shard_xy(g, p, px, py);
    L.gpix = (uint32_t)(py * sc.width + px);
    mega_sample<COUNT, true>(L, sc, g, root, cnt);
    return true;
}

#if defined(__HIPCC__)
__shared__ int spec_hint_lds[4];
__device__ __forceinline__ void spec_hint_set() { spec_hint_lds[threadIdx.x >> 6] = 1; }
__device__ __forceinline__ bool spec_hint_take() {
    const bool h = spec_hint_lds[threadIdx.x >> 6] != 0;
    spec_hint_lds[threadIdx.x >> 6] = 0;
    return h;
}
#else
inline thread_local bool g_spec_hint[4096];
inline void spec_hint_set() { g_spec_hint[(mega_slot() >> 6) & 4095] = true; }
inline bool spec_hint_take() {
    bool &h = g_spec_hint[(mega_slot() >> 6) & 4095];
    const bool v = h;
    h = false;
    return v;
}
#endif

template <bool CHAIN = false, class ML>
__device__ void spec_job_end(ML &L, const DevScene &sc, const ShardGeom &g, const WfState &st, int spp,
                             float *out, const NodeRec &root, V3 color, LaneCtr c,
                             const unsigned long long *queue = nullptr);

template <bool COUNT, bool FAST = false, bool CHAIN = false, class Stack, class ML>
__device__ __forceinline__ void mega_shade(ML &L, const DevScene &sc, const ShardGeom &g, const WfState &st,
                                           int spp, float *out, unsigned *cost, const NodeRec &root, Stack &stk,
                                           Counters &cnt, bool tail = false, bool park = false,
                                           const unsigned long long *queue = nullptr) {
    LaneRec P{st.rec_ab, st.rec_c, mega_slot_of(L), st.lanes, V3{0.f, 0.f, 0.f}, 0, false};
    Hit h = L.T.best;
    LaneCtr c = lane_ctr(L);
    bool next = false;
    const bool shaded = h.prim >= 0 && h.t < sc.max_distance;
    if (shaded) {
#if defined(__HIPCC__)
        if constexpr (kUvRecompute) {
            RT_CHECK(h.prim < sc.n_tris, 1, h.prim, h.prim = 0);
            hit_uv(sc, L.r, h);
        }
#endif
        Rng rng = lane_rng(L);
        const bool cont = shade_hit<COUNT>(sc, L.r, h, rng, cnt, P, c.nv, stk);
        lane_rng_set(L, rng);
        if (cont && c.power > 0) {
            c.power -= 1;
            next = true;
        }
    }
    if constexpr (FAST) P.flush_e();
    if (next) {
        lane_ctr_set(L, c);
        mega_begin<COUNT>(L, root, cnt);
        return;
    }
    if (!COUNT && !FAST && tail) {
        spec_job_end<CHAIN>(L, sc, g, st, spp, out, root, fold_path(P, c.nv, shaded), c, queue);
        return;
    }
    const V3 sm = rtv::add(lane_sum(L), fold_path(P, c.nv, !FAST && shaded));
    lane_sum_set(L, sm);
    if (++c.s == (FAST ? L.send : spp)) {
        const long long o = FAST ? L.dst : L.pix;
        out[3 * o + 0] = sm.x;
        out[3 * o + 1] = sm.y;
        out[3 * o + 2] = sm.z;
        if (COUNT && cost) cost[L.pix] = (unsigned)(cnt.aabb + cnt.tri + cnt.laabb + cnt.ltri - L.work0);
        if constexpr (CHAIN && !FAST) chain_store(chain_of(queue), (uint32_t)L.pix, (uint32_t)c.s, lane_rng(L), sm);
        L.pix = -1;
        L.state = M_IDLE;
        return;
    }
    if (!COUNT && !FAST && park) {
        lane_ctr_set(L, c);
        L.state = M_IDLE;
        return;
    }
    lane_ctr_set(L, c);
    mega_sample<COUNT, FAST>(L, sc, g, root, cnt);
}


template <bool COUNT, class Stack, class TS>
__device__ __forceinline__ bool light_step(const DevScene &sc, const Ray &r, TS &T, Stack &stk, Counters &cnt,
                                           const float4 *dir_rec) {
    const uint32_t id = stk.get(--T.sp).x;
    const NodeRec nd = load_node(sc.light_node, id);
    if ((nd.b & 3u) == 3u) {
        const uint32_t first = nd.a, count = nd.b >> 2;
        for (uint32_t k = first; k < first + count; ++k) {
            const float4 a = sc.light[4 * k], b = sc.light[4 * k + 1], c = sc.light[4 * k + 2], w = sc.light[4 * k + 3];
            TriHit h;
            if (COUNT) cnt.ltri++;
            if (tri_hit(V3{a.x, a.y, a.z}, V3{a.w, b.x, b.y}, V3{b.z, b.w, c.x}, r, h)) {
                V3 n{c.y, c.z, c.w};
                if (rtv::dot(r.d, n) > 0) n = rtv::neg(n);
                const float4 dq = *dir_rec;
                const float probability = 1.f / w.x;
                T.acc += fabsf(probability * (h.t * h.t) / rtv::dot(n, V3{dq.x, dq.y, dq.z}));
            }
        }
    } else {
        const uint32_t left = nd.a;
        float e;
        const NodeRec l = load_node(sc.light_node, left), rr = load_node(sc.light_node, left + 1);
        if (COUNT) cnt.laabb += 2;
        const bool hl = aabb_hit(l.mn, l.mx, r, e);
        const bool hr = aabb_hit(rr.mn, rr.mx, r, e);
        RT_CHECK(T.sp + 2 <= kStack, 13, T.sp, T.sp = 0);
        if (hr) stk.put(T.sp++, make_uint2(left + 1, 0u));
        if (hl) stk.put(T.sp++, make_uint2(left, 0u));
    }
    return T.sp == 0;
}

template <bool COUNT, bool FAST, class Stack, class ML>
__device__ __forceinline__ void mega_shade_split(ML &L, const DevScene &sc, const ShardGeom &g,
                                                 const WfState &st, int spp, float *out, unsigned *cost,
                                                 const NodeRec &root, Stack &stk, Counters &cnt) {
    const long long slot = mega_slot();
    LaneRec P{st.rec_ab, st.rec_c, slot, st.lanes, V3{0.f, 0.f, 0.f}, 0, false};
    float4 *mid = st.mid + slot;
    const long long ln = st.lanes;
    LaneCtr c = lane_ctr(L);
    bool next = false;
    if (L.state == M_READY) {
        const Hit h = L.T.best;
        ShadeMid m;
        bool pre = false;
        if (h.prim >= 0 && h.t < sc.max_distance) {
            Rng rng = lane_rng(L);
            pre = shade_pre<COUNT>(sc, L.r, h, rng, cnt, P, c.nv, m);
            lane_rng_set(L, rng);
        }
        if (pre) {
            if (sc.n_lights) {
                P.flush_e();
                mid[0] = make_float4(m.pos.x, m.pos.y, m.pos.z, m.r2);
                mid[ln] = make_float4(m.N.x, m.N.y, m.N.z, m.metallic);
                mid[2 * ln] = make_float4(m.dir.x, m.dir.y, m.dir.z, __int_as_float(m.mesh));
                mid[3 * ln] = make_float4(L.r.d.x, L.r.d.y, L.r.d.z, m.tc.x);
                mid[4 * ln] = make_float4(m.tc.y, 0.f, 0.f, 0.f);
                if (COUNT) cnt.lq++;
                L.r = make_ray(m.pos, m.dir);
                L.T.acc = 0.f;
                L.T.sp = 0;
                stk.put(L.T.sp++, make_uint2(0u, 0u));
                L.state = M_LTRAV;
                lane_ctr_set(L, c);
                return;
            }
            next = shade_post(sc, L.r.d, m, scene_pdf_lp(sc, m.N, rtv::neg(L.r.d), m.r2, m.dir, 0.f), P, c.nv, L.r) &&
                   c.power > 0;
        }
    } else {
        const float4 q0 = mid[0], q1 = mid[ln], q2 = mid[2 * ln], q3 = mid[3 * ln], q4 = mid[4 * ln];
        ShadeMid m;
        m.pos = V3{q0.x, q0.y, q0.z};
        m.r2 = q0.w;
        m.N = V3{q1.x, q1.y, q1.z};
        m.metallic = q1.w;
        m.dir = V3{q2.x, q2.y, q2.z};
        m.mesh = __float_as_int(q2.w);
        m.tc = V2{q3.w, q4.x};
        const V3 rd{q3.x, q3.y, q3.z};
        P.set_e(c.nv - 1, P.get_e(c.nv - 1));
        const float lp = L.T.acc / (float)sc.n_lights;
        next = shade_post(sc, rd, m, scene_pdf_lp(sc, m.N, rtv::neg(rd), m.r2, m.dir, lp), P, c.nv, L.r) && c.power > 0;
    }
    if (next) c.power -= 1;
    P.flush_e();
    if (next) {
        lane_ctr_set(L, c);
        mega_begin<COUNT>(L, root, cnt);
        return;
    }
    const V3 sm = rtv::add(lane_sum(L), fold_path(P, c.nv));
    lane_sum_set(L, sm);
    if (++c.s == (FAST ? L.send : spp)) {
        const long long o = FAST ? L.dst : L.pix;
        out[3 * o + 0] = sm.x;
        out[3 * o + 1] = sm.y;
        out[3 * o + 2] = sm.z;
        if (COUNT && cost) cost[L.pix] = (unsigned)(cnt.aabb + cnt.tri + cnt.laabb + cnt.ltri - L.work0);
        L.pix = -1;
        L.state = M_IDLE;
        return;
    }
    lane_ctr_set(L, c);
    mega_sample<COUNT, FAST>(L, sc, g, root, cnt);
}

template <bool COUNT, class Stack, class Nodes, bool FAST = false, bool LSPLIT = false, bool CHAIN = false, class ML>
__device__ __forceinline__ void mega_iterate(ML &L, bool shade_now, const DevScene &sc, const ShardGeom &g,
                                             const WfState &st, int spp, float *out, unsigned *cost,
                                             const NodeRec &root, Stack &stk, const Nodes &nodes, Counters &cnt,
                                             bool tail = false, bool park = false,
                                             const unsigned long long *queue = nullptr) {
    if constexpr (LSPLIT) {
        if (shade_now) {
            if (L.state == M_READY || L.state == M_LREADY)
                mega_shade_split<COUNT, FAST>(L, sc, g, st, spp, out, cost, root, stk, cnt);
            return;
        }
        if (L.state == M_LTRAV) {
            if (light_step<COUNT>(sc, L.r, L.T, stk, cnt, st.mid + 2 * st.lanes + mega_slot())) L.state = M_LREADY;
            return;
        }
    }
    if (shade_now) {
        if (L.state == M_READY)
            mega_shade<COUNT, FAST, CHAIN>(L, sc, g, st, spp, out, cost, root, stk, cnt, tail, park, queue);
    } else if (L.state == M_TRAV) {
        if (trav_step<COUNT>(sc, L.r, L.T, stk, nodes, cnt)) L.state = M_READY;
    }
}


#if defined(RT_MEGA_PROF) && defined(__HIPCC__)
__device__ unsigned long long g_spec_prof[16];
__shared__ unsigned long long spec_prof_lds[16];
#define RT_SPEC_STAT(k, v) atomicAdd(&::rtd::spec_prof_lds[k], (unsigned long long)(v))
__shared__ unsigned long long spec_wave_t0_lds[4];
constexpr int kChainRec = 1 << 20;
__device__ unsigned long long g_chain_t[kChainRec];
__device__ unsigned int g_chain_pix[kChainRec];
__device__ unsigned int g_chain_n;
#define RT_SPEC_CHAIN_END(spp, pix) \
    RT_SPEC_STAT(14, (wall_clock64() - ::rtd::spec_wave_t0_lds[threadIdx.x >> 6]) / (unsigned long long)(spp)); \
    RT_SPEC_STAT(15, 1); \
    { \
        const unsigned ci_ = atomicAdd(&::rtd::g_chain_n, 1u); \
        if (ci_ < (unsigned)::rtd::kChainRec) { \
            ::rtd::g_chain_t[ci_] = wall_clock64(); \
            ::rtd::g_chain_pix[ci_] = (unsigned)(pix); \
        } \
    }
#elif !defined(__HIPCC__)
inline unsigned long long g_spec_prof[16];
#define RT_SPEC_STAT(k, v) (::rtd::g_spec_prof[k] += (unsigned long long)(v))
#define RT_SPEC_CHAIN_END(spp, pix) do { } while (0)
#else
#define RT_SPEC_STAT(k, v) do { } while (0)
#define RT_SPEC_CHAIN_END(spp, pix) do { } while (0)
#endif

#ifndef RT_SPEC_WINDOW
#define RT_SPEC_WINDOW 3
#endif
#ifndef RT_SPEC_ISSUE
#define RT_SPEC_ISSUE 2
#endif
constexpr uint32_t kRecActive = 1u;
constexpr uint32_t kRecXf = 2u;
constexpr int kSpecWindow = RT_SPEC_WINDOW;
#ifndef RT_SPEC_LAZY
#define RT_SPEC_LAZY 1
#endif
constexpr bool kSpecLazy = RT_SPEC_LAZY != 0;
constexpr int kSpecIssue = RT_SPEC_ISSUE;
static_assert(kSpecWindow >= 1 && kSpecWindow <= 10, "lane table holds 10 slots");
constexpr int kTabBits = 6;
constexpr unsigned long long kTabMask = (1ull << kTabBits) - 1ull;
__device__ __forceinline__ int spec_tab(unsigned long long t, int q) { return (int)((t >> (kTabBits * q)) & kTabMask); }
__device__ __forceinline__ unsigned long long spec_tab_set(unsigned long long t, int q, int ln) {
    return (t & ~(kTabMask << (kTabBits * q))) | ((unsigned long long)ln << (kTabBits * q));
}

struct SpecView {
    uint4 *base;
    long long lanes;
    long long wbase;
    __device__ __forceinline__ uint4 *w(int plane, int r) const { return base + ((long long)plane * lanes + wbase + r); }
};
__device__ __forceinline__ Rng rng_unpack(uint4 v) { return Rng{v.x, v.y, __uint_as_float(v.z)}; }
__device__ __forceinline__ bool rng_same(const Rng &a, const Rng &b) {
    return a.x == b.x && a.saved_avail == b.saved_avail && __float_as_uint(a.saved) == __float_as_uint(b.saved);
}
__device__ __forceinline__ uint4 v3_pack(V3 v, uint32_t w) {
    return make_uint4(__float_as_uint(v.x), __float_as_uint(v.y), __float_as_uint(v.z), w);
}
__device__ __forceinline__ bool job_state(int s) { return s != M_IDLE; }

#if defined(__HIPCC__)
__device__ __forceinline__ uint32_t wshfl(uint32_t v, int src) { return (uint32_t)__shfl((int)v, src, 64); }
template <class T> struct WArr;
template <> struct WArr<uint32_t> {
    uint32_t v;
    __device__ __forceinline__ uint32_t get(int) const { return v; }
    __device__ __forceinline__ void put(int, uint32_t x) { v = x; }
    __device__ __forceinline__ uint32_t at(int s) const { return wshfl(v, s); }
};
template <> struct WArr<int> {
    int v;
    __device__ __forceinline__ int get(int) const { return v; }
    __device__ __forceinline__ void put(int, int x) { v = x; }
    __device__ __forceinline__ int at(int s) const { return __shfl(v, s, 64); }
};
template <> struct WArr<Rng> {
    Rng v;
    __device__ __forceinline__ Rng get(int) const { return v; }
    __device__ __forceinline__ void put(int, Rng x) { v = x; }
    __device__ __forceinline__ Rng at(int s) const {
        return Rng{wshfl(v.x, s), wshfl(v.saved_avail, s), __uint_as_float(wshfl(__float_as_uint(v.saved), s))};
    }
};
template <> struct WArr<V3> {
    V3 v;
    __device__ __forceinline__ V3 get(int) const { return v; }
    __device__ __forceinline__ void put(int, V3 x) { v = x; }
    __device__ __forceinline__ V3 at(int s) const { return V3{__shfl(v.x, s, 64), __shfl(v.y, s, 64), __shfl(v.z, s, 64)}; }
};
#define WBALLOT(acc, lane, p) ((acc) = __ballot(p))
#define WAVE_PHASE(lane, ...)                   \
    {                                            \
        const int lane = (int)(threadIdx.x & 63); \
        __VA_ARGS__                              \
    }
struct SpecLanes {
    MegaLane &L;
    __device__ __forceinline__ MegaLane &operator[](int) const { return L; }
};
#else
template <class T> struct WArr {
    T v[64];
    T get(int l) const { return v[l]; }
    void put(int l, T x) { v[l] = x; }
    T at(int s) const { return v[s]; }
};
#define WBALLOT(acc, lane, p) ((acc) |= (p) ? (1ull << (lane)) : 0ull)
#define WAVE_PHASE(lane, ...) \
    for (int lane = 0; lane < 64; ++lane) { __VA_ARGS__ }
struct SpecLanes {
    MegaLane *W;
    MegaLane &operator[](int l) const { return W[l]; }
};
#endif

#ifndef RT_SPEC_PRIO
#define RT_SPEC_PRIO 1
#endif
constexpr bool kSpecPrio = RT_SPEC_PRIO != 0;

#if defined(__HIPCC__)
__device__ __forceinline__ void wave_order(const WArr<uint32_t> &key, WArr<int> &srec, WArr<int> &rank) {
    const int lane = (int)(threadIdx.x & 63);
    uint32_t k = key.v;
#pragma unroll
    for (int b = 2; b <= 64; b <<= 1)
#pragma unroll
        for (int j = b >> 1; j > 0; j >>= 1) {
            const uint32_t o = (uint32_t)__shfl_xor((int)k, j, 64);
            const bool keep_min = ((lane & j) == 0) == ((lane & b) == 0);
            k = keep_min ? (o < k ? o : k) : (o > k ? o : k);
        }
    srec.v = (int)(k & 63u);
    rank.v = __builtin_amdgcn_ds_permute(srec.v << 2, lane);
}
#else
inline void wave_order(const WArr<uint32_t> &key, WArr<int> &srec, WArr<int> &rank) {
    uint32_t k[64];
    for (int l = 0; l < 64; ++l) k[l] = key.get(l);
    std::sort(k, k + 64);
    for (int p = 0; p < 64; ++p) {
        srec.put(p, (int)(k[p] & 63u));
// ... 406 lines not shown
```

### raytracing-hw_amd/csrc/rt_path.h

```cpp
#pragma once
#include <cstdint>
#if defined(__HIPCC__)
#include <hip/hip_runtime.h>
#else
#include <cmath>
#include <cstring>
#define __device__
#define __host__
#define __forceinline__ inline
struct float4 { float x, y, z, w; };
struct uint2 { uint32_t x, y; };
struct uint4 { uint32_t x, y, z, w; };
inline uint2 make_uint2(uint32_t a, uint32_t b) { return {a, b}; }
inline uint4 make_uint4(uint32_t a, uint32_t b, uint32_t c, uint32_t d) { return {a, b, c, d}; }
inline uint32_t __float_as_uint(float f) { uint32_t u; std::memcpy(&u, &f, 4); return u; }
inline float __uint_as_float(uint32_t u) { float f; std::memcpy(&f, &u, 4); return f; }
inline int __float_as_int(float f) { int u; std::memcpy(&u, &f, 4); return u; }
inline float __int_as_float(int u) { float f; std::memcpy(&f, &u, 4); return f; }
inline float4 make_float4(float a, float b, float c, float d) { return {a, b, c, d}; }
using std::isnan;
#endif

#include "rt_libm.h"
#include "rt_srgb_lut.h"
#include "rt_vec.h"

#if defined(RT_DEBUG_CHECKS) && defined(__HIPCC__)
__device__ unsigned long long rt_debug_word;
__device__ int rt_debug_poison;
__device__ unsigned rt_debug_prints;
#define RT_CHECK(cond, code, val, fix)                                                                        \
    do {                                                                                                     \
        if (!(cond)) {                                                                                       \
            atomicCAS(&rt_debug_word, 0ull, ((unsigned long long)(code) << 56) | ((unsigned long long)(val) & 0xffffffffffffffull)); \
            fix;                                                                                             \
        }                                                                                                    \
    } while (0)
#else
#define RT_CHECK(cond, code, val, fix) do { } while (0)
#endif

#if defined(RT_MEGA_PROF) && defined(__HIPCC__)
__shared__ unsigned long long rt_prof_lds[8];
#define RT_PROF_BEGIN long long rt_pt_ = clock64();
#define RT_PROF_SEG(k)                                                                                   \
    do {                                                                                                 \
        const long long t1_ = clock64();                                                                 \
        if ((int)(threadIdx.x & 63) == __ffsll((unsigned long long)__ballot(1)) - 1)                     \
            atomicAdd(&rt_prof_lds[k], (unsigned long long)(t1_ - rt_pt_));                              \
        rt_pt_ = t1_;                                                                                    \
    } while (0)
#else
#define RT_PROF_BEGIN
#define RT_PROF_SEG(k) do { } while (0)
#endif

namespace rtd {

using rtv::V2;
using rtv::V3;
using rtv::V4;

constexpr int kMaxDepth = 16;
constexpr int kStack = 64;
constexpr float kPiF = 3.14159265358979323846f;
constexpr float kInvPiF = 0.318309886183790671538f;
constexpr float kStep = 1e-4f;
constexpr float kRoughness2Limit = 0.03f;

inline void fill_decode_lut(float *lut) {
    for (int b = 0; b < 256; ++b) {
        lut[b] = rtm::kSrgbLut[b];
        lut[256 + b] = (float)b / 255.f;
    }
}

__device__ __forceinline__ float unorm8(uint32_t b) {
    constexpr float r = 0x1.010102p-8f;
    const float x = (float)b, q = x * r;
    return __builtin_fmaf(__builtin_fmaf(-q, 255.f, x), r, q);
}
__device__ __forceinline__ float texel_decode(const float *lut, uint32_t byte, bool srgb) {
#if defined(__HIP_DEVICE_COMPILE__)
    const float s = lut[byte], l = unorm8(byte);
    return srgb ? s : l;
#else
    return lut[(srgb ? 0u : 256u) + byte];
#endif
}

struct DevScene {
    const float4 *tri;
    const float4 *tri_attr;
    const float4 *tri_tan;
    const float4 *node;
    const float4 *light;
    const float4 *light_node;
    const float *mesh_f;
    const int *mesh_tex;
    const double *mesh_nt;
    const uint4 *tex_info;
    const uint32_t *texels;
    const float *lut;
    int n_lights;
    int n_tris, n_nodes, n_meshes;
    int ray_depth;
    float max_distance;
    int width, height;
    float fwidth, fheight;
    float cam_pos[3];
    float cam_axes[9];
    float tan_fov[2];
};

struct Counters {
    uint32_t rays, aabb, tri, lq, laabb, ltri, hits;
};

struct Rng {
    uint32_t x;
    uint32_t saved_avail;
    float saved;
};

constexpr uint32_t kFastKey = 0x5eed2026u;
__host__ __device__ __forceinline__ uint4 philox4x32_10(uint4 c, uint2 k) {
    for (int r = 0; r < 10; ++r) {
        if (r) {
            k.x += 0x9E3779B9u;
            k.y += 0xBB67AE85u;
        }
        const uint64_t p0 = (uint64_t)0xD2511F53u * c.x, p1 = (uint64_t)0xCD9E8D57u * c.z;
        c = make_uint4((uint32_t)(p1 >> 32) ^ c.y ^ k.x, (uint32_t)p1, (uint32_t)(p0 >> 32) ^ c.w ^ k.y, (uint32_t)p0);
    }
    return c;
}
__host__ __device__ __forceinline__ uint32_t fast_sample_seed(uint32_t pixel, uint32_t sample) {
    const uint32_t w = philox4x32_10(make_uint4(sample, 0u, 0u, 0u), make_uint2(pixel, kFastKey)).x % 2147483647u;
    return w == 0 ? 1u : w;
}

__device__ __forceinline__ uint32_t rng_next(Rng &r) {
    uint64_t t = (uint64_t)r.x * 48271u;
    uint32_t v = (uint32_t)(t & 0x7fffffffu) + (uint32_t)(t >> 31);
    if (v >= 0x7fffffffu) v -= 0x7fffffffu;
    r.x = v;
    return v;
}
__device__ __forceinline__ float rng_canonical(Rng &r) {
    float s = (float)(rng_next(r) - 1u);
    float v = s / 2147483648.0f;
    if (v >= 1.0f) v = 0x1.fffffep-1f;
    return v;
}
__device__ __forceinline__ float rng_uniform_m11(Rng &r) { return rng_canonical(r) * 2.0f + (-1.0f); }
__device__ __forceinline__ float rng_offset(Rng &r) { return rng_canonical(r) * 1.0f + (-0.5f); }
__device__ __forceinline__ float rng_normal(Rng &r) {
    float ret;
    if (r.saved_avail) {
        r.saved_avail = 0;
        ret = r.saved;
    } else {
        float x, y, r2;
        do {
            x = 2.0f * rng_canonical(r) - 1.0f;
            y = 2.0f * rng_canonical(r) - 1.0f;
            r2 = x * x + y * y;
        } while (r2 > 1.0f || r2 == 0.0f);
        const float mult = sqrtf(-2.0f * rtm::logf_glibc(r2) / r2);
        r.saved = x * mult;
        r.saved_avail = 1;
        ret = y * mult;
    }
    return ret * 1.0f + 0.0f;
}

struct Ray {
    V3 o, d, inv;
};
__device__ __forceinline__ Ray make_ray(V3 p, V3 dir) {
    Ray r;
    r.o = p;
    r.d = rtv::normal(dir);
    r.inv = rtv::divv(V3{1.f, 1.f, 1.f}, r.d);
    return r;
}

__device__ __forceinline__ bool aabb_hit(const float mn[3], const float mx[3], const Ray &r, float &dist) {
    const float o[3] = {r.o.x, r.o.y, r.o.z};
    const float d[3] = {r.d.x, r.d.y, r.d.z};
    const float inv[3] = {r.inv.x, r.inv.y, r.inv.z};
    bool inside = true;
    int quad[3];
    float cand[3];
#pragma unroll
    for (int i = 0; i < 3; ++i) {
        if (o[i] < mn[i]) { quad[i] = 0; cand[i] = mn[i]; inside = false; }
        else if (o[i] > mx[i]) { quad[i] = 2; cand[i] = mx[i]; inside = false; }
        else { quad[i] = 1; cand[i] = 0.f; }
    }
    if (inside) { dist = 0.f; return true; }
    float maxT[3];
#pragma unroll
    for (int i = 0; i < 3; ++i) maxT[i] = (quad[i] != 1 && d[i] != 0.f) ? (cand[i] - o[i]) * inv[i] : -1.f;
    int wp = 0;
    if (maxT[wp] < maxT[1]) wp = 1;
    if (maxT[wp] < maxT[2]) wp = 2;
    const float tw = maxT[wp];
    if (tw < 0.f) return false;
    float coord[3];
#pragma unroll
    for (int i = 0; i < 3; ++i) {
        if (wp != i) {
            coord[i] = o[i] + tw * d[i];
            if (coord[i] < mn[i] || coord[i] > mx[i]) return false;
        } else {
            coord[i] = cand[i];
        }
    }
    dist = rtv::length(rtv::sub(V3{coord[0], coord[1], coord[2]}, r.o));
    return true;
}

struct TriHit {
    float t, u, v;
};
__device__ __forceinline__ bool tri_hit(V3 v0, V3 U, V3 V, const Ray &r, TriHit &h) {
    V3 p = rtv::cross(r.d, V);
    float det = rtv::dot(U, p);
    if (-1e-6 < (double)det && (double)det < 1e-6) return false;
    float inv_det = 1.f / det;
    V3 s = rtv::sub(r.o, v0);
    float u = inv_det * rtv::dot(s, p);
    if (u < 0 || u > 1) return false;
    V3 q = rtv::cross(s, U);
    float v = inv_det * rtv::dot(r.d, q);
    if (v < 0 || u + v > 1) return false;
    float t = inv_det * rtv::dot(V, q);
    if (t < 0.f) return false;
    h.t = t;
    h.u = u;
    h.v = v;
    return true;
}

__device__ __forceinline__ void load_tri(const float4 *tri, int id, V3 &v0, V3 &U, V3 &V) {
    float4 a = tri[3 * id], b = tri[3 * id + 1], c = tri[3 * id + 2];
    v0 = V3{a.x, a.y, a.z};
    U = V3{a.w, b.x, b.y};
    V = V3{b.z, b.w, c.x};
}

struct NodeRec {
    float mn[3], mx[3];
    uint32_t a, b;
};
__device__ __forceinline__ NodeRec load_node(const float4 *nodes, uint32_t id) {
    float4 p = nodes[2 * id], q = nodes[2 * id + 1];
    NodeRec n;
    n.mn[0] = p.x; n.mn[1] = p.y; n.mn[2] = p.z;
    n.mx[0] = p.w; n.mx[1] = q.x; n.mx[2] = q.y;
    n.a = __float_as_uint(q.z);
    n.b = __float_as_uint(q.w);
    return n;
}

struct Hit {
    float t, u, v;
    int prim;
};

template <bool COUNT>
__device__ bool closest_hit(const DevScene &sc, const Ray &r, Hit &best, Counters &cnt) {
    if (COUNT) { cnt.rays++; cnt.aabb++; }
    NodeRec nd = load_node(sc.node, 0);
    float e;
    if (!aabb_hit(nd.mn, nd.mx, r, e)) return false;
    uint2 stk[kStack];
    int sp = 0;
    uint32_t cur = 0;
    int phase = 0;
    float acc = 1e9f;
    best.t = 1e9f;
    best.prim = -1;
    const float dcomp[3] = {r.d.x, r.d.y, r.d.z};
    for (;;) {
        bool descend = false;
        if ((nd.b & 3u) == 3u) {
            const uint32_t first = nd.a, count = nd.b >> 2;
            for (uint32_t k = first; k < first + count; ++k) {
                V3 v0, U, V;
                load_tri(sc.tri, (int)k, v0, U, V);
                TriHit h;
                if (COUNT) cnt.tri++;
                if (tri_hit(v0, U, V, r, h)) {
                    if (h.t < acc) acc = h.t;
                    if (h.t < best.t) { best.t = h.t; best.u = h.u; best.v = h.v; best.prim = (int)k; }
                }
            }
        } else {
            const uint32_t left = nd.a;
            const bool left_first = dcomp[nd.b] > 0;
            if (phase == 0) {
                const uint32_t c0 = left_first ? left : left + 1;
                NodeRec cn = load_node(sc.node, c0);
                if (COUNT) cnt.aabb++;
                if (aabb_hit(cn.mn, cn.mx, r, e)) {
                    stk[sp++] = make_uint2(cur | (1u << 31), __float_as_uint(acc));
                    cur = c0; phase = 0; acc = 1e9f; nd = cn;
                    descend = true;
                } else {
                    phase = 1;
                }
            }
            if (!descend && phase == 1) {
                const uint32_t c1 = left_first ? left + 1 : left;
                NodeRec cn = load_node(sc.node, c1);
                if (COUNT) cnt.aabb++;
                if (aabb_hit(cn.mn, cn.mx, r, e) && !(e > acc)) {
                    stk[sp++] = make_uint2(cur, __float_as_uint(acc));
                    cur = c1; phase = 0; acc = 1e9f; nd = cn;
                    descend = true;
                }
            }
        }
        if (descend) continue;
        if (sp == 0) break;
        uint2 f = stk[--sp];
        const float pacc = __uint_as_float(f.y);
        acc = acc < pacc ? acc : pacc;
        phase = (f.x >> 31) ? 1 : 2;
        cur = f.x & 0x7fffffffu;
        nd = load_node(sc.node, cur);
        if (phase == 2) {
        }
    }
    return best.prim >= 0;
}

template <bool COUNT, class Stack>
__device__ float light_pdf(const DevScene &sc, V3 point, V3 direction, Counters &cnt, Stack &stk) {
    if (COUNT) cnt.lq++;
    Ray r = make_ray(point, direction);
    int sp = 0;
    stk.put(sp++, make_uint2(0u, 0u));
    float prob = 0.f;
    while (sp > 0) {
        const uint32_t id = stk.get(--sp).x;
        NodeRec nd = load_node(sc.light_node, id);
        if ((nd.b & 3u) == 3u) {
            const uint32_t first = nd.a, count = nd.b >> 2;
            for (uint32_t k = first; k < first + count; ++k) {
                float4 a = sc.light[4 * k], b = sc.light[4 * k + 1], c = sc.light[4 * k + 2], w = sc.light[4 * k + 3];
                TriHit h;
                if (COUNT) cnt.ltri++;
                if (tri_hit(V3{a.x, a.y, a.z}, V3{a.w, b.x, b.y}, V3{b.z, b.w, c.x}, r, h)) {
                    V3 n{c.y, c.z, c.w};
                    if (rtv::dot(r.d, n) > 0) n = rtv::neg(n);
                    const float probability = 1.f / w.x;
                    prob += fabsf(probability * (h.t * h.t) / rtv::dot(n, direction));
                }
            }
        } else {
            const uint32_t left = nd.a;
            float e;
            NodeRec l = load_node(sc.light_node, left), rr = load_node(sc.light_node, left + 1);
            if (COUNT) cnt.laabb += 2;
            const bool hl = aabb_hit(l.mn, l.mx, r, e);
            const bool hr = aabb_hit(rr.mn, rr.mx, r, e);
            RT_CHECK(sp + 2 <= kStack, 13, sp, sp = 0);
            if (hr) stk.put(sp++, make_uint2(left + 1, 0u));
            if (hl) stk.put(sp++, make_uint2(left, 0u));
        }
    }
    return prob / (float)sc.n_lights;
}
struct LocalStack {
    uint32_t id[kStack];
    __device__ __forceinline__ void put(int i, uint2 v) { id[i] = v.x; }
    __device__ __forceinline__ uint2 get(int i) const { return make_uint2(id[i], 0u); }
};
template <bool COUNT>
__device__ float light_pdf(const DevScene &sc, V3 point, V3 direction, Counters &cnt) {
    LocalStack stk;
    return light_pdf<COUNT>(sc, point, direction, cnt, stk);
}

__device__ __forceinline__ V4 tex_sample_ti(const DevScene &sc, const uint4 ti, V2 p, bool srgb) {
    const int W = (int)ti.y, H = (int)ti.z;
    p.x -= floorf(p.x);
    p.y -= floorf(p.y);
    p.x *= (float)W;
    p.y *= (float)H;
    const int px = (int)floorf(p.x), py = (int)floorf(p.y);
    const float dx = p.x - floorf(p.x), dy = p.y - floorf(p.y);
    uint32_t texel[4];
    auto wrap = [](int v, int n) {
        v = v >= n ? v - n : v;
        return v >= n ? v - n : v;
    };
#pragma unroll
    for (int ddy = 0; ddy < 2; ++ddy)
#pragma unroll
        for (int ddx = 0; ddx < 2; ++ddx) {
            const int x = wrap(px + ddx, W), y = wrap(py + ddy, H);
#ifdef __HIPCC__
            const uint32_t idx = (uint32_t)(((y >> 2) * ((W + 3) >> 2) + (x >> 2)) * 16 + (y & 3) * 4 + (x & 3));
#else
            const uint32_t idx = (uint32_t)(y * W + x);
#endif
            texel[ddx * 2 + ddy] = sc.texels[ti.x + idx];
        }
    float res[4];
#pragma unroll
    for (int c = 0; c < 4; ++c) {
        float v[4];
#pragma unroll
        for (int k = 0; k < 4; ++k) {
            const uint32_t byte = (texel[k] >> (8 * c)) & 0xffu;
            v[k] = texel_decode(sc.lut, byte, srgb);
        }
        res[c] = v[0] * (1 - dx) * (1 - dy) + v[1] * (1 - dx) * dy + v[2] * dx * (1 - dy) + v[3] * dx * dy;
    }
    return V4{res[0], res[1], res[2], res[3]};
}
__device__ __forceinline__ V4 tex_sample(const DevScene &sc, int tex, V2 p, bool srgb) {
    return tex_sample_ti(sc, sc.tex_info[tex], p, srgb);
}

__device__ __forceinline__ V3 sphere(Rng &r) {
    float a = rng_normal(r);
    float b = rng_normal(r);
    float c = rng_normal(r);
    return rtv::normal(V3{a, b, c});
}
__device__ __forceinline__ V3 cosine_sample(V3 n, Rng &r) {
    V3 d;
    do {
        d = rtv::add(sphere(r), n);
    } while ((double)rtv::length(d) < 1e-12);
    return rtv::normal(d);
}
__device__ __forceinline__ float cosine_pdf(V3 n, V3 d) { return rtv::smax(0.f, rtv::dot(d, n)) * kInvPiF; }

__device__ __forceinline__ void disc_draw(Rng &r, float &ux, float &uy) {
    do {
        ux = rng_uniform_m11(r);
        uy = rng_uniform_m11(r);
    } while (ux * ux + uy * uy > 1.f);
}

__device__ __forceinline__ V3 vndf_sample(V3 n, V3 eye, float alpha, Rng &r) {
    const V3 Z{0.f, 0.f, 1.f};
    V4 rot = rtv::quat_from_two_vectors(n, Z);
    V3 Ve = rtv::rotate(eye, rot);
    V3 Vh = rtv::normal(V3{Ve.x * alpha, Ve.y * alpha, Ve.z});
    float lensq = Vh.x * Vh.x + Vh.y * Vh.y;
    V3 T1 = lensq > 0 ? rtv::mul(V3{-Vh.y, Vh.x, 0}, 1.f / sqrtf(lensq)) : V3{1, 0, 0};
    V3 T2 = rtv::cross(Vh, T1);
    float ux, uy;
    disc_draw(r, ux, uy);
    float s = 0.5f + 0.5f * Vh.z;
    float ty = (1.f - s) * sqrtf(1.f - ux * ux) + s * uy;
    V3 Nh = rtv::add(rtv::add(rtv::mul(T1, ux), rtv::mul(T2, ty)),
                     rtv::mul(Vh, sqrtf(rtv::smax(0.f, 1.f - ux * ux - ty * ty))));
    V3 Ne = rtv::normal(V3{alpha * Nh.x, alpha * Nh.y, rtv::smax(0.f, Nh.z)});
    Ne = rtv::rotate(Ne, rtv::conj(rot));
    return rtv::normal(rtv::sub(rtv::mul(rtv::mul(Ne, 2.f), rtv::dot(Ne, eye)), eye));
}
__device__ __forceinline__ float vndf_pdf(V3 n, V3 eye, float alpha, V3 dir) {
    const V3 Z{0.f, 0.f, 1.f};
    V4 rot = rtv::quat_from_two_vectors(n, Z);
    V3 sn = rtv::normal(rtv::add(dir, eye));
    V3 V = rtv::rotate(eye, rot);
    V3 Ni = rtv::rotate(sn, rot);
    if (rtv::dot(V, Ni) < 0.f) return 0.f;
    float alpha2 = alpha * alpha;
    float q = Ni.x * Ni.x / alpha2 + Ni.y * Ni.y / alpha2 + Ni.z * Ni.z;
    float invD = (float)((double)(kPiF * alpha * alpha) * ((double)q * (double)q));
    float invG1 = 0.5f + 0.5f * sqrtf(1.f + (alpha2 * V.x * V.x + alpha2 * V.y * V.y) / (V.z * V.z));
    return 1.f / (4.f * invD * invG1 * rtv::dot(V, Z));
}
__device__ __forceinline__ V3 light_sample(const DevScene &sc, V3 point, Rng &r) {
    int s = (int)floorf((rng_uniform_m11(r) + 1.f) * 0.5f * (float)sc.n_lights);
    if (s == sc.n_lights) s -= 1;
    float4 a = sc.light[4 * s], b = sc.light[4 * s + 1], c = sc.light[4 * s + 2];
    float u = (rng_uniform_m11(r) + 1.f) / 2;
    float v = (rng_uniform_m11(r) + 1.f) / 2;
    if (u + v > 1) { u = 1 - u; v = 1 - v; }
    V3 res = rtv::add(rtv::add(V3{a.x, a.y, a.z}, rtv::mul(V3{a.w, b.x, b.y}, u)), rtv::mul(V3{b.z, b.w, c.x}, v));
    return rtv::normal(rtv::sub(res, point));
}

__device__ __forceinline__ float ggx(float alpha, V3 N, V3 H) {
    float alpha2 = alpha * alpha;
    float NdotH = rtv::dot(N, H);
    return alpha2 * kInvPiF / ((NdotH * NdotH * (alpha2 - 1) + 1) * (NdotH * NdotH * (alpha2 - 1) + 1));
}
__device__ __forceinline__ float smith(float alpha, V3 N, V3 V, V3 L) {
    float alpha2 = alpha * alpha;
    if (rtv::dot(N, L) <= 0 || rtv::dot(N, V) <= 0) return 0;
    float nd[2] = {fabsf(rtv::dot(N, L)), fabsf(rtv::dot(N, V))};
    float res = 1.f;
#pragma unroll
    for (int k = 0; k < 2; ++k) res *= 2 * nd[k] / (nd[k] + sqrtf(alpha2 + (1 - alpha2) * nd[k] * nd[k]));
    return res;
}

__device__ __forceinline__ V3 mul_vector_d(const double *m, V3 t) {
    const float tv[4] = {t.x, t.y, t.z, 0.f};
    float res[3] = {0.f, 0.f, 0.f};
#pragma unroll 1
    for (int j = 0; j < 4; ++j) {
        const double tj = (double)tv[j];
#pragma unroll
        for (int i = 0; i < 3; ++i) res[i] = (float)((double)res[i] + m[4 * j + i] * tj);
    }
    return V3{res[0], res[1], res[2]};
}

struct PathRec {
    V3 e[kMaxDepth], m[kMaxDepth];
    float coeff[kMaxDepth], cosv[kMaxDepth], alpha[kMaxDepth];
    __device__ __forceinline__ void set_e(int k, V3 v) { e[k] = v; }
    __device__ __forceinline__ void set_brdf(int k, V3 mm, float c, float cs, float a) {
        m[k] = mm;
        coeff[k] = c;
        cosv[k] = cs;
        alpha[k] = a;
    }
    __device__ __forceinline__ V3 get_e(int k) const { return e[k]; }
    __device__ __forceinline__ V3 get_m(int k) const { return m[k]; }
    __device__ __forceinline__ float get_coeff(int k) const { return coeff[k]; }
    __device__ __forceinline__ float get_cos(int k) const { return cosv[k]; }
    __device__ __forceinline__ float get_alpha(int k) const { return alpha[k]; }
};

struct SoARec {
    float *base;
    long long n;
// ... 32 lines not shown
    float x, y, r2;
    do {
        x = 2.0f * rng_canonical(r) - 1.0f;
        y = 2.0f * rng_canonical(r) - 1.0f;
        r2 = x * x + y * y;
    } while (r2 > 1.0f || r2 == 0.0f);
    gen = true;
    lx = x;
    lr2 = r2;
    r.saved_avail = 1;
}
__device__ __forceinline__ void rng_skip_sample(Rng &r, int k, int n_lights) {
    (void)rng_next(r);
    (void)rng_next(r);
    bool gen = false;
    float lx = 0.f, lr2 = 1.f;
    for (int v = 0; v < k; ++v) {
        const int b = mixture_pick(r, n_lights);
        if (b == 0) {
            rng_normal_skip(r, gen, lx, lr2);
            rng_normal_skip(r, gen, lx, lr2);
            rng_normal_skip(r, gen, lx, lr2);
        } else if (b == 1) {
            float ux, uy;
            disc_draw(r, ux, uy);
        } else {
            (void)rng_next(r);
            (void)rng_next(r);
            (void)rng_next(r);
        }
    }
    if (gen) {
        const float mult = sqrtf(-2.0f * rtm::logf_glibc(lr2) / lr2);
        r.saved = lx * mult;
    }
}

template <bool COUNT, class Stack>
__device__ __forceinline__ float scene_pdf(const DevScene &sc, V3 pos, V3 N, V3 eye, float r2, V3 dir, Counters &cnt,
                                           Stack &stk) {
    if (!sc.n_lights) return (cosine_pdf(N, dir) + vndf_pdf(N, eye, r2, dir)) / 2;
    return (cosine_pdf(N, dir) + light_pdf<COUNT>(sc, pos, dir, cnt, stk) + vndf_pdf(N, eye, r2, dir)) / 3;
}
template <bool COUNT>
__device__ __forceinline__ float scene_pdf(const DevScene &sc, V3 pos, V3 N, V3 eye, float r2, V3 dir, Counters &cnt) {
    LocalStack stk;
    return scene_pdf<COUNT>(sc, pos, N, eye, r2, dir, cnt, stk);
}

struct AosRec {
    float4 *ab;
    float *c;
    long long i;
    int D;
    V3 e;
    int ek;
    bool pending;
    __device__ __forceinline__ long long v(int k) const { return i * D + k; }
    __device__ __forceinline__ void set_e(int k, V3 x) { e = x; ek = k; pending = true; }
    __device__ __forceinline__ void set_brdf(int k, V3 mm, float cf, float cs, float a) {
        ab[2 * v(k)] = make_float4(e.x, e.y, e.z, cf);
        ab[2 * v(k) + 1] = make_float4(mm.x, mm.y, mm.z, cs);
        c[v(k)] = a;
        pending = false;
    }
    __device__ __forceinline__ void flush_e() {
        if (pending) ab[2 * v(ek)] = make_float4(e.x, e.y, e.z, 0.f);
        pending = false;
    }
    __device__ __forceinline__ V3 get_e(int k) const { const float4 a = ab[2 * v(k)]; return V3{a.x, a.y, a.z}; }
    __device__ __forceinline__ V3 get_m(int k) const { const float4 b = ab[2 * v(k) + 1]; return V3{b.x, b.y, b.z}; }
    __device__ __forceinline__ float get_coeff(int k) const { return ab[2 * v(k)].w; }
    __device__ __forceinline__ float get_cos(int k) const { return ab[2 * v(k) + 1].w; }
    __device__ __forceinline__ float get_alpha(int k) const { return c[v(k)]; }
};

#ifndef RT_REC_NT
#define RT_REC_NT 0
#endif
__device__ __forceinline__ void rec_st(float4 &dst, float4 v) {
#if RT_REC_NT && defined(__HIP_DEVICE_COMPILE__)
    typedef float v4f __attribute__((ext_vector_type(4)));
    const v4f x = {v.x, v.y, v.z, v.w};
    __builtin_nontemporal_store(x, reinterpret_cast<v4f *>(&dst));
#else
    dst = v;
#endif
}
__device__ __forceinline__ float4 rec_ld(const float4 &src) {
#if RT_REC_NT && defined(__HIP_DEVICE_COMPILE__)
    typedef float v4f __attribute__((ext_vector_type(4)));
    const v4f x = __builtin_nontemporal_load(reinterpret_cast<const v4f *>(&src));
    return make_float4(x.x, x.y, x.z, x.w);
#else
    return src;
#endif
}
struct LaneRec {
    float4 *R;
    float *al;
    long long i, lanes;
    V3 e;
    int ek;
    bool pending;
    __device__ __forceinline__ uint32_t v(int k) const { return (uint32_t)k * (uint32_t)lanes + (uint32_t)i; }
    __device__ __forceinline__ float4 &rec(uint32_t vk, int half) const {
        return *(float4 *)((char *)R + (size_t)((vk << 5) + (uint32_t)(16 * half)));
    }
    __device__ __forceinline__ float &alp(uint32_t vk) const { return *(float *)((char *)al + (size_t)(vk << 2)); }
    __device__ __forceinline__ void set_e(int k, V3 x) { e = x; ek = k; pending = true; }
    __device__ __forceinline__ void set_brdf(int k, V3 mm, float cf, float cs, float a) {
        const bool one = __float_as_uint(a) == 0x3f800000u;
        rec_st(rec(v(k), 0), make_float4(__uint_as_float(__float_as_uint(cf) | (one ? 0u : 0x80000000u)), mm.x, mm.y, mm.z));
        rec_st(rec(v(k), 1), make_float4(cs, e.x, e.y, e.z));
        if (!one) alp(v(k)) = a;
        pending = false;
    }
    __device__ __forceinline__ void flush_e() {
        if (pending) rec_st(rec(v(ek), 1), make_float4(0.f, e.x, e.y, e.z));
        pending = false;
    }
    __device__ __forceinline__ V3 get_e(int k) const { const float4 b = rec_ld(rec(v(k), 1)); return V3{b.y, b.z, b.w}; }
};
__device__ __forceinline__ V3 fold_path(const LaneRec &P, int nv, bool last_here = false) {
    if (nv == 0) return V3{0.f, 0.f, 0.f};
    V3 c = P.e;
    if (!last_here) {
        const float4 last = rec_ld(P.rec(P.v(nv - 1), 1));
        c = V3{last.y, last.z, last.w};
    }
    for (int hi = nv - 2; hi >= 0; hi -= 4) {
        float4 A[4], B[4];
#pragma unroll
        for (int j = 0; j < 4; ++j) {
            const int k = hi - j >= 0 ? hi - j : 0;
            A[j] = rec_ld(P.rec(P.v(k), 0));
            B[j] = rec_ld(P.rec(P.v(k), 1));
        }
#pragma unroll
        for (int j = 0; j < 4; ++j) {
            if (hi - j < 0) break;
            const uint32_t cb = __float_as_uint(A[j].x);
            const float alpha = (cb >> 31) ? P.alp(P.v(hi - j)) : 1.f;
            V3 x = rtv::mul(c, __uint_as_float(cb & 0x7fffffffu));
            x = rtv::mulv(x, V3{A[j].y, A[j].z, A[j].w});
            x = rtv::mul(x, B[j].x);
            x = rtv::mul(x, alpha);
            c = rtv::add(V3{B[j].y, B[j].z, B[j].w}, x);
        }
    }
    return c;
}

struct ShadeMid {
    V3 pos, N, dir;
    V2 tc;
    float r2, metallic;
    int mesh;
};

template <bool COUNT, class Rec>
__device__ __forceinline__ bool shade_pre(const DevScene &sc, const Ray &r, const Hit &hit, Rng &rng, Counters &cnt,
                                          Rec &P, int &nv, ShadeMid &m) {
    RT_PROF_BEGIN
    if (COUNT) cnt.hits++;
    int id = hit.prim;
    RT_CHECK(id >= 0 && id < sc.n_tris, 1, id, id = 0);
    RT_CHECK(nv >= 0 && nv < kMaxDepth - 1, 2, nv, nv = 0);
    const float u = hit.u, v = hit.v;
    const float4 t2 = sc.tri[3 * id + 2];
    V3 ngeo{t2.y, t2.z, t2.w};
    bool inside = false;
    if (rtv::dot(r.d, ngeo) > 0) { inside = true; ngeo = rtv::neg(ngeo); }
    const float4 a0 = sc.tri_attr[4 * id], a1 = sc.tri_attr[4 * id + 1], a2 = sc.tri_attr[4 * id + 2],
                 a3 = sc.tri_attr[4 * id + 3];
    int mesh = __float_as_int(a3.w);
    RT_CHECK(mesh >= 0 && mesh < sc.n_meshes, 3, mesh, mesh = 0);
    const float *mf = sc.mesh_f + 12 * mesh;
    const int *mt = sc.mesh_tex + 4 * mesh;
    const int mt_e = mt[3], mt_n = mt[1], mt_mr = mt[2];
    const uint4 ti_e = sc.tex_info[mt_e >= 0 ? mt_e : 0], ti_n = sc.tex_info[mt_n >= 0 ? mt_n : 0],
                ti_mr = sc.tex_info[mt_mr >= 0 ? mt_mr : 0];
#ifdef __HIPCC__
    asm volatile("" ::"v"(ti_e.x), "v"(ti_n.x), "v"(ti_mr.x));
#endif
    const float w = 1 - u - v;
    const V2 tc{w * a2.y + u * a2.w + v * a3.y, w * a2.z + u * a3.x + v * a3.z};
    V3 emission{mf[3], mf[4], mf[5]};
    if (mt_e >= 0) emission = rtv::mulv(rtv::reduce(tex_sample_ti(sc, ti_e, tc, true)), emission);
    P.set_e(nv, emission);
    RT_PROF_SEG(0);
    V3 n0{a0.x, a0.y, a0.z}, n1{a0.w, a1.x, a1.y}, n2{a1.z, a1.w, a2.x};
    V3 lz = rtv::normal(rtv::add(rtv::add(rtv::mul(n0, w), rtv::mul(n1, u)), rtv::mul(n2, v)));
    V3 N = lz;
    if (mt_n >= 0) {
        const float4 g0 = sc.tri_tan[3 * id], g1 = sc.tri_tan[3 * id + 1], g2 = sc.tri_tan[3 * id + 2];
        V3 t0{g0.x, g0.y, g0.z}, t1{g1.x, g1.y, g1.z}, tt2{g2.x, g2.y, g2.z};
        V3 lx = rtv::normal(mul_vector_d(sc.mesh_nt + 16 * mesh,
                                         rtv::normal(rtv::add(rtv::add(rtv::mul(t0, w), rtv::mul(t1, u)), rtv::mul(tt2, v)))));
        V3 ly = rtv::mul(rtv::cross(lz, lx), g0.w);
        V3 s = rtv::reduce(tex_sample_ti(sc, ti_n, tc, false));
        V3 ln = rtv::mul(rtv::addf(s, -0.5f), 2.f);
        N = rtv::normal(rtv::add(rtv::add(rtv::mul(lx, ln.x), rtv::mul(ly, ln.y)), rtv::mul(lz, ln.z)));
    }
    if (inside) N = rtv::neg(N);
    RT_PROF_SEG(1);
    float r2 = mf[7], metallic = mf[6];
    if (mt_mr >= 0) {
        V4 mr = tex_sample_ti(sc, ti_mr, tc, false);
        float rr = mr.y * mr.y;
        r2 = rr * mf[7];
        metallic = mr.z * mf[6];
    }
    r2 = rtv::smax(kRoughness2Limit, r2);
    const V3 pos = rtv::add(r.o, rtv::mul(r.d, hit.t));
    const V3 eye = rtv::neg(r.d);
    RT_PROF_SEG(2);
    const V3 dir = scene_sample(sc, pos, N, eye, r2, rng);
    RT_PROF_SEG(3);
    nv++;
    if (rtv::dot(dir, N) <= 0.f) {
        if (rtv::dot(dir, ngeo) <= 0.f) return false;
        N = ngeo;
    }
    m.pos = pos;
    m.N = N;
    m.dir = dir;
    m.tc = tc;
    m.r2 = r2;
    m.metallic = metallic;
    m.mesh = mesh;
    return true;
}

__device__ __forceinline__ float scene_pdf_lp(const DevScene &sc, V3 N, V3 eye, float r2, V3 dir, float lp) {
    if (!sc.n_lights) return (cosine_pdf(N, dir) + vndf_pdf(N, eye, r2, dir)) / 2;
    return (cosine_pdf(N, dir) + lp + vndf_pdf(N, eye, r2, dir)) / 3;
}

template <class Rec>
__device__ __forceinline__ bool shade_post(const DevScene &sc, const V3 rd, const ShadeMid &m, float pdf, Rec &P, int nv,
                                           Ray &r_out) {
    RT_PROF_BEGIN
    if (pdf <= 0.f || isnan(pdf)) return false;
    const V3 pos = m.pos, N = m.N, dir = m.dir, eye = rtv::neg(rd);
    const V2 tc = m.tc;
    const float r2 = m.r2, metallic = m.metallic;
    const float *mf = sc.mesh_f + 12 * m.mesh;
    const int *mt = sc.mesh_tex + 4 * m.mesh;
    const float coeff = 1 / pdf;
    const V3 half = rtv::normal(rtv::sub(dir, rd));
    const float vis = smith(r2, N, eye, dir) * (1.f / (4 * fabsf(rtv::dot(N, rd)) * fabsf(rtv::dot(N, dir))));
    const float spec = ggx(r2, N, half) * vis;
    const float VdotH = fabsf(rtv::dot(eye, half));
    V3 base{mf[0], mf[1], mf[2]};
    if (mt[0] >= 0) base = rtv::mulv(rtv::reduce(tex_sample(sc, mt[0], tc, true)), base);
    const float p5 = rtm::pow5_glibc(1.f - VdotH);
    const V3 fres{base.x + (1.f - base.x) * p5, base.y + (1.f - base.y) * p5, base.z + (1.f - base.z) * p5};
    const V3 metal = rtv::mul(fres, spec);
    const V3 diffuse = rtv::mul(base, kInvPiF);
    const float dsc = 0.04f + (1.f - 0.04f) * p5;
    const V3 dielectric = rtv::add(rtv::mul(diffuse, 1 - dsc), rtv::mul(rtv::mul(V3{1.f, 1.f, 1.f}, spec), dsc));
    P.set_brdf(nv - 1, rtv::add(rtv::mul(dielectric, 1 - metallic), rtv::mul(metal, metallic)), coeff,
               rtv::dot(dir, N), mf[8]);
    r_out = make_ray(rtv::add(pos, rtv::mul(dir, kStep)), dir);
    RT_PROF_SEG(5);
    return true;
}


template <bool COUNT, class Rec, class Stack>
__device__ bool shade_hit(const DevScene &sc, Ray &r, const Hit &hit, Rng &rng, Counters &cnt, Rec &P, int &nv,
                          Stack &stk) {
    ShadeMid m;
    if (!shade_pre<COUNT>(sc, r, hit, rng, cnt, P, nv, m)) return false;
    RT_PROF_BEGIN
    const float pdf = scene_pdf<COUNT>(sc, m.pos, m.N, rtv::neg(r.d), m.r2, m.dir, cnt, stk);
    RT_PROF_SEG(4);
    return shade_post(sc, r.d, m, pdf, P, nv, r);
}
template <bool COUNT, class Rec>
__device__ bool shade_hit(const DevScene &sc, Ray &r, const Hit &hit, Rng &rng, Counters &cnt, Rec &P, int &nv) {
    LocalStack stk;
    return shade_hit<COUNT>(sc, r, hit, rng, cnt, P, nv, stk);
}

template <class Rec>
__device__ __forceinline__ V3 fold_path(const Rec &P, int nv) {
    if (nv == 0) return V3{0.f, 0.f, 0.f};
    V3 c = P.get_e(nv - 1);
    for (int k = nv - 2; k >= 0; --k) {
        V3 x = rtv::mul(c, P.get_coeff(k));
        x = rtv::mulv(x, P.get_m(k));
        x = rtv::mul(x, P.get_cos(k));
        x = rtv::mul(x, P.get_alpha(k));
        c = rtv::add(P.get_e(k), x);
    }
    return c;
}

__device__ __forceinline__ V3 fold_path(const AosRec &P, int nv) {
    if (nv == 0) return V3{0.f, 0.f, 0.f};
    V3 c = P.get_e(nv - 1);
    for (int hi = nv - 2; hi >= 0; hi -= 4) {
        float4 A[4], B[4];
        float C[4];
#pragma unroll
        for (int j = 0; j < 4; ++j) {
            const int k = hi - j >= 0 ? hi - j : 0;
            A[j] = P.ab[2 * P.v(k)];
            B[j] = P.ab[2 * P.v(k) + 1];
            C[j] = P.c[P.v(k)];
        }
#pragma unroll
        for (int j = 0; j < 4; ++j) {
            if (hi - j < 0) break;
            V3 x = rtv::mul(c, A[j].w);
            x = rtv::mulv(x, V3{B[j].x, B[j].y, B[j].z});
            x = rtv::mul(x, B[j].w);
            x = rtv::mul(x, C[j]);
            c = rtv::add(V3{A[j].x, A[j].y, A[j].z}, x);
        }
    }
    return c;
}

template <bool COUNT>
__device__ V3 trace_sample(const DevScene &sc, Ray r, Rng &rng, Counters &cnt) {
    PathRec P;
    int nv = 0;
    int power = sc.ray_depth;
    while (power > 0) {
        power -= 1;
        Hit hit;
        bool ok = closest_hit<COUNT>(sc, r, hit, cnt);
        if (!(ok && hit.t < sc.max_distance)) break;
        if (!shade_hit<COUNT>(sc, r, hit, rng, cnt, P, nv)) break;
    }
    return fold_path(P, nv);
}

__device__ __forceinline__ Ray camera_ray(const DevScene &sc, int px, int py, float ox, float oy) {
    V3 t;
    t.x = (2.f * ((float)px + 0.5f + ox) / sc.fwidth - 1) * sc.tan_fov[0];
    t.y = -(2.f * ((float)py + 0.5f + oy) / sc.fheight - 1) * sc.tan_fov[1];
    t.z = 1;
    V3 d{0.f, 0.f, 0.f};
    const float tv[3] = {t.x, t.y, t.z};
#pragma unroll
    for (int i = 0; i < 3; ++i)
        d = rtv::add(d, rtv::mul(V3{sc.cam_axes[3 * i], sc.cam_axes[3 * i + 1], sc.cam_axes[3 * i + 2]}, tv[i]));
    return make_ray(V3{sc.cam_pos[0], sc.cam_pos[1], sc.cam_pos[2]}, d);
}

template <bool COUNT>
__device__ V3 render_pixel(const DevScene &sc, int i, int j, int spp, Counters &cnt) {
    Rng rng;
    uint32_t seed = (uint32_t)(j * sc.width + i) % 2147483647u;
    rng.x = seed == 0 ? 1u : seed;
    rng.saved_avail = 0;
    rng.saved = 0.f;
    V3 sum{0.f, 0.f, 0.f};
    for (int s = 0; s < spp; ++s) {
        float ox = rng_offset(rng);
        float oy = rng_offset(rng);
        Ray r = camera_ray(sc, i, j, ox, oy);
        V3 c = trace_sample<COUNT>(sc, r, rng, cnt);
        sum = rtv::add(sum, c);
    }
    return sum;
}

}
```

### raytracing-hw_amd/csrc/rt_wavefront.h

```cpp
#pragma once
#include "rt_path.h"

namespace rtd {

struct ShardGeom {
    int width, rank, world, row_block;
    long long n_pixels;
    uint32_t wm, rbm;
    int ws, rbs;
};
__device__ __forceinline__ int div_magic(int n, uint32_t m, int s) {
    return (int)(((unsigned long long)(uint32_t)n * m) >> s);
}
inline void div_magic_make(uint32_t d, uint32_t &m, int &s) {
    int l = 0;
    while ((1ull << l) < d) ++l;
    s = 31 + l;
    m = (uint32_t)(((1ull << s) + d - 1) / d);
}
inline ShardGeom shard_geom(int width, int rank, int world, int row_block, long long n_pixels) {
    ShardGeom g{width, rank, world, row_block, n_pixels, 0u, 0u, 0, 0};
    div_magic_make((uint32_t)width, g.wm, g.ws);
    div_magic_make((uint32_t)row_block, g.rbm, g.rbs);
    return g;
// ... 335 lines not shown
template <bool DIST2 = kFarDist2, class Stack, class TS>
__device__ __forceinline__ bool trav_pop(TS &T, Stack &stk) {
    float acc = T.acc;
    int sp = T.sp;
    double thr = DIST2 ? far_thr(acc) : 0.0;
    for (int n = 0;; ++n) {
        if (sp == 0) {
            T.sp = 0;
            T.acc = acc;
            return true;
        }
        if (kMaxPops > 0 && n == kMaxPops) {
            T.sp = sp;
            T.acc = acc;
            return false;
        }
        const uint2 f = stk.get(--sp);
        if (f.x == kFrameAcc) {
            const float p = __uint_as_float(f.y);
            acc = acc < p ? acc : p;
            if (DIST2) thr = far_thr(acc);
            continue;
        }
        const float e = __uint_as_float(f.y);
        if (!(DIST2 ? far_gt_thr(e, thr) : e > acc)) {
            stk.put(sp++, make_uint2(kFrameAcc, __float_as_uint(acc)));
#ifdef RT_STACK_PROBE
            RT_STACK_PROBE(sp);
#endif
            T.sp = sp;
            T.acc = 1e9f;
            trav_enter(T, f.x >> 10, f.x & 1023u);
            return false;
        }
    }
}

template <bool COUNT, bool DIST2 = kFarDist2, class Stack, class TS>
__device__ __forceinline__ void node_step(const float4 q[4], const Ray &r, TS &T, Stack &stk, Counters &cnt) {
    NodeRec L, R;
    L.mn[0] = q[0].x; L.mn[1] = q[0].y; L.mn[2] = q[0].z; L.mx[0] = q[0].w; L.mx[1] = q[1].x; L.mx[2] = q[1].y;
    L.a = __float_as_uint(q[1].z); L.b = __float_as_uint(q[1].w);
    R.mn[0] = q[2].x; R.mn[1] = q[2].y; R.mn[2] = q[2].z; R.mx[0] = q[2].w; R.mx[1] = q[3].x; R.mx[2] = q[3].y;
    R.a = __float_as_uint(q[3].z); R.b = __float_as_uint(q[3].w);
    if (COUNT) cnt.aabb += 2;
    const uint32_t dpos = (r.d.x > 0.f ? 1u : 0u) | (r.d.y > 0.f ? 2u : 0u) | (r.d.z > 0.f ? 4u : 0u);
    const bool lf = (dpos >> T.b) & 1u;
    float cF[3];
    bool hL, hR, inF;
    box_pair_hit(L, R, r, lf, hL, hR, cF, inF);
    const float ef = DIST2 ? box_dist2(cF, inF, r) : box_dist(cF, inF, r);
    const bool hn = lf ? hL : hR, hf = lf ? hR : hL;
    const uint32_t na = lf ? L.a : R.a, nb = lf ? L.b : R.b, fa = lf ? R.a : L.a, fb = lf ? R.b : L.b;
    if (hn && hf) {
        RT_CHECK(T.sp < kStack, 11, T.sp, T.sp = 0);
        stk.put(T.sp++, make_uint2((fa << 10) | fb, __float_as_uint(ef)));
#ifdef RT_STACK_PROBE
        RT_STACK_PROBE(T.sp);
#endif
    }
    const bool far_only = !hn && hf && !(DIST2 ? ef > kFarMax2 : ef > 1e9f);
    if (hn || far_only) trav_enter(T, hn ? na : fa, hn ? nb : fb);
    else T.phase = TP_POP;
}

template <bool COUNT, bool DIST2 = kFarDist2, class Stack, class Nodes, class TS>
__device__ __forceinline__ bool trav_step(const DevScene &sc, const Ray &r, TS &T, Stack &stk,
                                          const Nodes &nodes, Counters &cnt) {
    constexpr int N = RT_LEAF_N;
    const bool at_node = T.phase == TP_NODE, at_leaf = T.phase == TP_LEAF;
    const uint32_t k = T.k, klast = T.kend - 1u;
    RT_CHECK(!at_node || T.a + 1 < (uint32_t)sc.n_nodes, 10, T.a, T.a = 0);
    RT_CHECK(!at_leaf || T.kend <= (uint32_t)sc.n_tris, 12, T.kend, T.k = T.kend = 1);
    float4 q[4 + 3 * (N - 1)];
    {
        const float4 *p0 = at_node ? nodes.pair(T.a) : sc.tri + 3 * (size_t)(at_leaf ? k : 0u);
#pragma unroll
        for (int i = 0; i < 4; ++i) q[i] = p0[i];
#pragma unroll
        for (int j = 1; j < N; ++j) {
            const uint32_t kj = at_leaf ? (k + j < klast ? k + j : klast) : 0u;
            const float4 *pj = sc.tri + 3 * (size_t)kj;
#pragma unroll
            for (int i = 0; i < 3; ++i) q[4 + 3 * (j - 1) + i] = pj[i];
        }
#ifdef __HIPCC__
        asm volatile("" ::"v"(q[0].x), "v"(q[1].y), "v"(q[2].z), "v"(q[3].w));
#endif
    }
    if (at_node) {
        node_step<COUNT, DIST2>(q, r, T, stk, cnt);
    } else if (at_leaf) {
#pragma unroll
        for (int j = 0; j < N; ++j) {
            const int o = j == 0 ? 0 : 4 + 3 * (j - 1);
            const V3 v0{q[o].x, q[o].y, q[o].z}, U{q[o].w, q[o + 1].x, q[o + 1].y}, V{q[o + 1].z, q[o + 1].w, q[o + 2].x};
            const bool valid = j == 0 || k + j <= klast;
            TriHit h;
            const bool hit = tri_hit_bl(v0, U, V, r, h) & valid;
            if (COUNT && valid) cnt.tri++;
            if (hit) {
                T.acc = h.t < T.acc ? h.t : T.acc;
                if (h.t < T.best.t) { T.best.t = h.t; T.best.u = h.u; T.best.v = h.v; T.best.prim = (int)(k + j); }
            }
        }
        T.k = k + N;
        if (T.k >= T.kend) T.phase = TP_POP;
    }
    if (T.phase == TP_POP) return trav_pop<DIST2>(T, stk);
    return false;
}

#ifdef __HIPCC__
#ifndef RT_LDS_STACK
#define RT_LDS_STACK 12
#endif
#ifndef RT_SPEC_LDS_STACK
#define RT_SPEC_LDS_STACK 15
#endif
constexpr int kLdsStack = RT_LDS_STACK;
constexpr int kLdsStackSpec = RT_SPEC_LDS_STACK;
constexpr int kLdsStackWf = 11;
template <int K>
__device__ __forceinline__ uint2 *lds_stack_frames() {
    __shared__ uint2 frames[K * 256];
    return frames;
}
template <int K>
struct LdsStackT {
    static_assert(K >= 1 && K < kStack, "LDS frames");
    uint2 *spill;
    __device__ __forceinline__ void put(int i, uint2 v) {
        if (i < K) lds_stack_frames<K>()[i * 256 + threadIdx.x] = v;
        else spill[i - K] = v;
    }
    __device__ __forceinline__ uint2 get(int i) const {
        uint2 v;
        if (i < K) {
            v = lds_stack_frames<K>()[i * 256 + threadIdx.x];
        } else {
            v = spill[i - K];
            asm volatile("" : "+v"(v.x), "+v"(v.y));
        }
        return v;
    }
};


#ifndef RT_UV_RECOMPUTE
#define RT_UV_RECOMPUTE 1
#endif
constexpr bool kUvRecompute = RT_UV_RECOMPUTE != 0;

__device__ __forceinline__ void hit_uv(const DevScene &sc, const Ray &r, Hit &h) {
    const float4 *t = sc.tri + 3 * (size_t)h.prim;
    const float4 t0 = t[0], t1 = t[1], t2 = t[2];
    TriHit th;
    tri_hit_bl(V3{t0.x, t0.y, t0.z}, V3{t0.w, t1.x, t1.y}, V3{t1.z, t1.w, t2.x}, r, th);
    h.u = th.u;
    h.v = th.v;
}

template <int CTL>
__device__ __forceinline__ void quad_min_step(float &c, float &cu, float &cv, int &cj) {
    const float c2 = __int_as_float(__builtin_amdgcn_mov_dpp(__float_as_int(c), CTL, 0xF, 0xF, false));
    const int j2 = __builtin_amdgcn_mov_dpp(cj, CTL, 0xF, 0xF, false);
    const bool take = c2 < c || (c2 == c && j2 < cj);
    if (!kUvRecompute) {
        const float u2 = __int_as_float(__builtin_amdgcn_mov_dpp(__float_as_int(cu), CTL, 0xF, 0xF, false));
        const float v2 = __int_as_float(__builtin_amdgcn_mov_dpp(__float_as_int(cv), CTL, 0xF, 0xF, false));
        cu = take ? u2 : cu;
        cv = take ? v2 : cv;
    }
    c = take ? c2 : c;
    cj = take ? j2 : cj;
}


struct NoHook {
    __device__ __forceinline__ void operator()() const {}
};
#ifndef RT_LEAF_DEFER
#define RT_LEAF_DEFER 6
#endif
#ifndef RT_LEAF_DEFER_MAX
#define RT_LEAF_DEFER_MAX 4
#endif
constexpr int kLeafDefer = RT_LEAF_DEFER, kLeafDeferMax = RT_LEAF_DEFER_MAX;
#ifndef RT_PLAIN_LEAF_DEFER
#define RT_PLAIN_LEAF_DEFER 6
#endif
constexpr int kLeafDeferPlain = RT_PLAIN_LEAF_DEFER;
template <bool COUNT, int kCoopLeaves, bool MASK_LOAD, int DEFER = kLeafDefer, bool DIST2 = kFarDist2, class Stack,
          class Nodes, class TS, class Hook = NoHook>
__device__ __forceinline__ bool trav_step_coop(const DevScene &sc, const Ray &r, TS &T, Stack &stk,
                                               const Nodes &nodes, Counters &cnt, bool active, int round_min,
                                               const Hook &hook = Hook{}, int *leaf_defer = nullptr) {
    static_assert(kCoopLeaves >= 1 && kCoopLeaves <= 16, "4 helper lanes per leaf lane");
    __shared__ float4 wf_coop_rec[4][kCoopLeaves][2];
    const int lane = (int)(threadIdx.x & 63), wave = (int)(threadIdx.x >> 6);
    const bool at_node = active && T.phase == TP_NODE, at_leaf = active && T.phase == TP_LEAF;
    RT_CHECK(!at_node || T.a + 1 < (uint32_t)sc.n_nodes, 10, T.a, T.a = 0);
    RT_CHECK(!at_leaf || T.kend <= (uint32_t)sc.n_tris, 12, T.kend, T.k = T.kend = 1);
    float4 q[4];
    if (MASK_LOAD) {
        if (at_node) {
            const float4 *p0 = nodes.pair(T.a);
#pragma unroll
            for (int i = 0; i < 4; ++i) q[i] = p0[i];
        }
    } else {
        const float4 *p0 = nodes.pair(at_node ? T.a : 0u);
#pragma unroll
        for (int i = 0; i < 4; ++i) q[i] = p0[i];
    }
    const unsigned long long lm = __ballot(at_leaf);
    const int n_leaf = __popcll(lm);
    const int lrank = (int)__builtin_amdgcn_mbcnt_hi((uint32_t)(lm >> 32), __builtin_amdgcn_mbcnt_lo((uint32_t)lm, 0u));
    bool skip_leaves = false;
    if (DEFER > 0 && leaf_defer) {
        if (n_leaf > 0 && n_leaf < DEFER && *leaf_defer < kLeafDeferMax && __ballot(at_node) != 0ull) {
            skip_leaves = true;
            ++*leaf_defer;
        } else {
            *leaf_defer = 0;
        }
    }
    for (int base = 0; !skip_leaves && base < n_leaf; base += kCoopLeaves) {
        if (base > 0 && n_leaf - base < round_min) break;
        const int rank = lrank - base;
        const bool served = at_leaf && rank >= 0 && rank < kCoopLeaves;
        if (base > 0) __builtin_amdgcn_wave_barrier();
        if (served) {
            wf_coop_rec[wave][rank][0] = make_float4(r.o.x, r.o.y, r.o.z, __uint_as_float(T.k));
            wf_coop_rec[wave][rank][1] = make_float4(r.d.x, r.d.y, r.d.z, __uint_as_float(T.kend));
        }
        __builtin_amdgcn_fence(__ATOMIC_RELEASE, "wavefront");
        __builtin_amdgcn_wave_barrier();
        const int n_served = n_leaf - base < kCoopLeaves ? n_leaf - base : kCoopLeaves;
        const int h = lane >> 2, j = lane & 3;
        float c = __builtin_inff(), cu = 0.f, cv = 0.f;
        if (h < n_served) {
            const float4 a = wf_coop_rec[wave][h][0], b = wf_coop_rec[wave][h][1];
            const uint32_t k = __float_as_uint(a.w) + (uint32_t)j;
            if (k < __float_as_uint(b.w)) {
                const float4 *t = sc.tri + 3 * (size_t)k;
                const float4 t0 = t[0], t1 = t[1], t2 = t[2];
                Ray hr;
                hr.o = V3{a.x, a.y, a.z};
                hr.d = V3{b.x, b.y, b.z};
                TriHit th;
                if (tri_hit_bl(V3{t0.x, t0.y, t0.z}, V3{t0.w, t1.x, t1.y}, V3{t1.z, t1.w, t2.x}, hr, th) &&
                    th.t == th.t) {
                    c = th.t;
                    cu = th.u;
                    cv = th.v;
                }
            }
        }
        int cj = j;
        quad_min_step<0xB1>(c, cu, cv, cj);
        quad_min_step<0x4E>(c, cu, cv, cj);
        const int src = 4 * (served ? rank : 0);
        const float wc = __shfl(c, src, 64);
        const float wu = kUvRecompute ? 0.f : __shfl(cu, src, 64), wv = kUvRecompute ? 0.f : __shfl(cv, src, 64);
        const int wj = __shfl(cj, src, 64);
        if (served) {
            if (COUNT) cnt.tri += (T.kend - T.k < 4u ? T.kend - T.k : 4u);
            if (wc < T.acc) T.acc = wc;
            if (wc < T.best.t) {
                T.best.t = wc;
                if (!kUvRecompute) {
                    T.best.u = wu;
                    T.best.v = wv;
                }
                T.best.prim = (int)(T.k + (uint32_t)wj);
            }
            T.k += 4u;
            if (T.k >= T.kend) T.phase = TP_POP;
        }
    }
    hook();
    if (at_node) node_step<COUNT, DIST2>(q, r, T, stk, cnt);
    if (active && T.phase == TP_POP) return trav_pop<DIST2>(T, stk);
    return false;
}

#endif

template <bool COUNT>
__device__ __forceinline__ void closest_hit_wf(const DevScene &sc, const float4 *q, unsigned p, Hit &best, uint2 *stk,
                                               Counters &cnt) {
    uint32_t bits;
    int slot;
    const Ray r = load_qray_trav(q, p, bits, slot);
    const NodeRec root = load_node(sc.node, 0);
    TravState T;
    ArrayStack S{stk};
    const GlobalNodes nodes{sc.node};
    if (trav_start<COUNT>(bits, root.a, root.b, T, cnt))
        while (!trav_step<COUNT>(sc, r, T, S, nodes, cnt)) {
        }
    best = T.best;
}

__device__ __forceinline__ Ray start_sample(const DevScene &sc, const ShardGeom &g, long long i, Rng &rng, int &power) {
// ... 56 lines not shown
```

Measured before the change: 2059.

## Pack per-mesh material records and gather all texture taps up front in shading

Adds a packed 128-byte per-mesh material record that combines material floats, texture indices and texture descriptors. The plain megakernel shade path now loads the triangle, attributes, tangents and all four texture slots' texels in one early batch, instead of resolving dependent table lookups one after another. This is meant to cut serial memory latency chains in shading. The cost is higher register pressure from holding all taps live, which may lower occupancy; tangents are also fetched unconditionally when any mesh has a normal map. A self-check kernel validates the records.

```diff
diff --git a/raytracing-hw_amd/csrc/rt_device.hip b/raytracing-hw_amd/csrc/rt_device.hip
--- a/raytracing-hw_amd/csrc/rt_device.hip
+++ b/raytracing-hw_amd/csrc/rt_device.hip
@@ -17,6 +17,7 @@
 #include "rt_mega.h"
 #include "rt_quant_lut.h"
 #include "rt_scene.h"
+#include "rt_material.h"
 #include "rt_bvh_layout.h"
 #include "rt_launch_plan.h"
 #include "rt_select.h"
@@ -72,6 +73,14 @@
 #define RT_SPEC_FAR_DIST2 0
 #endif
 constexpr bool kPlainFarDist2 = RT_PLAIN_FAR_DIST2 != 0, kSpecFarDist2 = RT_SPEC_FAR_DIST2 != 0;
+#ifndef RT_PLAIN_SHADE_GATHER
+#define RT_PLAIN_SHADE_GATHER RT_SHADE_GATHER
+#endif
+#ifndef RT_SPEC_SHADE_GATHER
+#define RT_SPEC_SHADE_GATHER 0
+#endif
+constexpr int kPlainShade = RT_PLAIN_SHADE_GATHER ? rtd::SHADE_GATHER_HOLD : rtd::SHADE_TABLES,
+              kSpecShade = RT_SPEC_SHADE_GATHER ? rtd::SHADE_GATHER_HOLD : rtd::SHADE_TABLES;
 #ifndef RT_COOP_ROUND_MIN
 #define RT_COOP_ROUND_MIN 8
 #endif
@@ -91,13 +100,15 @@
 
 struct rt_device_blob {
     std::vector<uint8_t> bytes;
-    size_t o_tri, o_attr, o_tan, o_node, o_light, o_lnode, o_mf, o_mt, o_nt, o_ti, o_tx, o_lut;
+    size_t o_tri, o_attr, o_tan, o_node, o_light, o_lnode, o_mf, o_mt, o_nt, o_ti, o_tx, o_lut, o_mat;
+    size_t n_texels;
 };
 
 struct rt_device_scene {
     int device = -1;
     void *buf = nullptr;
     DevScene ds{};
+    size_t n_texels = 0;
     unsigned long long *counters = nullptr;
     unsigned long long *queue = nullptr;
     int cu_count = 0;
@@ -228,6 +239,7 @@
                unsigned long long *queue, const int *order, unsigned *cost, int cs, int mode) {
     constexpr bool kSpec = SPEC && !COUNT && !FAST && !LSPLIT;
     constexpr bool kChain = CHAIN && !COUNT && !FAST && !LSPLIT;
+    constexpr int kShade = kSpec ? kSpecShade : (!COUNT && !FAST && !LSPLIT && !kChain) ? kPlainShade : rtd::SHADE_TABLES;
     constexpr bool kFastChain = CHAIN && FAST && !COUNT && !LSPLIT && !SPEC;
     const int park_below = kFastChain ? 0 : rtp::mode_park_below(mode), resume_pct = kFastChain ? 0 : rtp::mode_resume_pct(mode);
     const uint4 *resume = kSpec && resume_pct > 0 ? (const uint4 *)queue[rtd::kQueueParkList] : nullptr;
@@ -450,16 +462,15 @@
             if (L.state == rtd::M_READY) {
                 L.T.phase = 0;
                 L.T.sp = 0;
-                rtd::mega_shade<COUNT, FAST, kChain>(L, sc, g, st, spp, out, cost, root, S, cnt, kSpec && tail, park, queue);
+                rtd::mega_shade<COUNT, FAST, kChain, kShade>(L, sc, g, st, spp, out, cost, root, S, cnt, kSpec && tail, park, queue);
             } else {
                 L.T.phase = (int)(pk & 3u);
                 L.state = (int)((pk >> 2) & 7u);
                 L.T.sp = (int)(pk >> 5);
             }
         } else {
-            rtd::mega_iterate<COUNT, decltype(S), decltype(nodes), FAST, LSPLIT, kChain>(L, shade_now, sc, g, st, spp, out,
-                                                                                       cost, root, S, nodes, cnt,
-                                                                                       kSpec && tail, false, queue);
+            rtd::mega_iterate<COUNT, decltype(S), decltype(nodes), FAST, LSPLIT, kChain, kShade>(
+                L, shade_now, sc, g, st, spp, out, cost, root, S, nodes, cnt, kSpec && tail, false, queue);
             if (kInvRecompute && shade_now) L.r.inv = rtv::divv(rtd::V3{1.f, 1.f, 1.f}, L.r.d);
         }
         if (kPackTrav && kInvRecompute && !LSPLIT && !kSpec && !FAST && shade_now)
@@ -725,26 +736,6 @@
     return off;
 }
 
-void tile_textures(const std::vector<uint32_t> &info, const std::vector<uint8_t> &texels, std::vector<uint32_t> &info_out,
-                   std::vector<uint32_t> &out) {
-    const size_t n = info.size() / 4;
-    info_out = info;
-    out.clear();
-    for (size_t t = 0; t < n; ++t) {
-        const uint32_t off = info[4 * t], w = info[4 * t + 1], h = info[4 * t + 2];
-        const uint32_t tw = (w + 3) / 4, th = (h + 3) / 4;
-        const size_t base = out.size();
-        info_out[4 * t] = (uint32_t)base;
-        out.resize(base + (size_t)tw * th * 16, 0u);
-        for (uint32_t y = 0; y < h; ++y)
-            for (uint32_t x = 0; x < w; ++x) {
-                uint32_t v;
-                std::memcpy(&v, &texels[4 * ((size_t)off + (size_t)y * w + x)], 4);
-                out[base + ((size_t)(y >> 2) * tw + (x >> 2)) * 16 + (y & 3) * 4 + (x & 3)] = v;
-            }
-    }
-}
-
 int ensure_blob(rt_scene *s) {
     if (s->blob) return RT_OK;
     if (s->bvh_depth + 2 >= (uint32_t)rtd::kStack || s->light_bvh_depth + 2 >= (uint32_t)rtd::kStack)
@@ -769,19 +760,33 @@
     b->o_mt = append(blob, s->mesh_tex);
     b->o_nt = append(blob, s->mesh_nt);
     std::vector<uint32_t> tinfo, tiled;
-    tile_textures(s->tex_info, s->texels, tinfo, tiled);
+    rtmat::tile_textures(s->tex_info, s->texels, tinfo, tiled);
     b->o_ti = append(blob, tinfo);
     b->o_tx = append(blob, tiled);
+    b->n_texels = tiled.size();
     std::vector<float> lut(512);
     rtd::fill_decode_lut(lut.data());
     b->o_lut = append(blob, lut);
+    std::vector<uint32_t> mat;
+    if (!rtmat::build_records(s->mesh_f.data(), s->mesh_tex.data(), s->mesh_f.size() / 12, tinfo.data(), tinfo.size() / 4, mat)) {
+        delete b;
+        return rt_fail(RT_ERR_FORMAT, "texture index out of range");
+    }
+    b->o_mat = append(blob, mat);
     blob.resize(rtp::align_up(blob.size()) + 256);
     s->blob = b;
     return RT_OK;
 }
 
+std::mutex g_live_mu;
+std::vector<rt_device_scene *> g_live;
+
 void free_device_scene(rt_device_scene *d) {
     if (!d) return;
+    {
+        std::lock_guard<std::mutex> lk(g_live_mu);
+        g_live.erase(std::remove(g_live.begin(), g_live.end(), d), g_live.end());
+    }
     DeviceGuard guard(d->device);
     if (guard.ok) {
         for (hipStream_t q : {d->fr.stream, d->fr.cp_stream})
@@ -845,6 +850,12 @@
     ds.tex_info = (const uint4 *)(base + b.o_ti);
     ds.texels = (const uint32_t *)(base + b.o_tx);
     ds.lut = (const float *)(base + b.o_lut);
+    d->n_texels = b.n_texels;
+#if RT_SHADE_GATHER
+    ds.mat = (const uint4 *)(base + b.o_mat);
+    ds.any_nmap = 0;
+    for (size_t m = 0; m < s->mesh_tex.size() / 4; ++m) ds.any_nmap |= s->mesh_tex[4 * m + 1] >= 0;
+#endif
     ds.n_lights = (int)(s->light.size() / 16);
     ds.n_tris = (int)(s->tri.size() / 12);
     ds.n_nodes = (int)(s->node.size() / 8);
@@ -859,6 +870,10 @@
     std::memcpy(ds.cam_axes, s->cam_axes, sizeof ds.cam_axes);
     std::memcpy(ds.tan_fov, s->tan_half_fov, sizeof ds.tan_fov);
     s->dev[device] = d;
+    {
+        std::lock_guard<std::mutex> lk(g_live_mu);
+        g_live.push_back(d);
+    }
     return RT_OK;
 }
 
@@ -2627,6 +2642,34 @@
     if ((threadIdx.x & 63) == 0 && local) atomicAdd(bad, local);
 }
 
+#if RT_SHADE_GATHER
+__global__ void __launch_bounds__(256) mat_check_kernel(rtd::DevScene sc, unsigned long long n_texels, unsigned long long *bad) {
+    unsigned long long local = 0;
+    for (int m = blockIdx.x * blockDim.x + threadIdx.x; m < sc.n_meshes; m += gridDim.x * blockDim.x) {
+        uint32_t r[32];
+        for (int q = 0; q < 8; ++q) {
+            const uint4 x = sc.mat[8 * m + q];
+            r[4 * q] = x.x; r[4 * q + 1] = x.y; r[4 * q + 2] = x.z; r[4 * q + 3] = x.w;
+        }
+        for (int k = 0; k < 12; ++k) local += r[k] != __float_as_uint(sc.mesh_f[12 * m + k]);
+        for (int k = 0; k < 4; ++k) {
+            const int t = sc.mesh_tex[4 * m + k];
+            local += r[rtmat::kRecTex + k] != (uint32_t)t;
+            uint4 ti = make_uint4(0u, 1u, 1u, 4u);
+            if (t >= 0) {
+                ti = sc.tex_info[t];
+                local += (unsigned long long)ti.x + (unsigned long long)((ti.y + 3) / 4) * ((ti.z + 3) / 4) * 16 > n_texels;
+            }
+            const uint32_t *d = r + rtmat::kRecDesc + 3 * k;
+            local += (d[0] != ti.x) + (d[1] != ti.y) + (d[2] != ti.z);
+        }
+        for (int k = 28; k < 32; ++k) local += r[k] != 0u;
+    }
+    for (int off = 32; off > 0; off >>= 1) local += __shfl_down(local, off, 64);
+    if ((threadIdx.x & 63) == 0 && local) atomicAdd(bad, local);
+}
+#endif
+
 __global__ void __launch_bounds__(256) far_check_kernel(unsigned long long *bad) {
     const uint32_t i = blockIdx.x * blockDim.x + threadIdx.x;
     unsigned long long local = 0;
@@ -2752,13 +2795,41 @@
         leaves[2 * (size_t)i + 1] = k0 + len;
     }
 }
+
+int mat_selfcheck(uint64_t *mismatches) {
+#if RT_SHADE_GATHER
+    std::lock_guard<std::mutex> lk(g_live_mu);
+    if (g_live.empty()) return rt_fail(RT_ERR_ARG, "rt_device_selfcheck 4: no scene is uploaded");
+    uint64_t total = 0;
+    for (rt_device_scene *ds : g_live) {
+        DeviceGuard guard(ds->device);
+        if (!guard.ok) return rt_fail(RT_ERR_DEVICE, "rt_device_selfcheck 4: hipSetDevice failed");
+        unsigned long long *d = nullptr, h = 0;
+        HIP_TRY(hipMalloc((void **)&d, sizeof *d));
+        hipError_t e = hipMemset(d, 0, sizeof *d);
+        if (e == hipSuccess) {
+            hipLaunchKernelGGL(mat_check_kernel, dim3(64), dim3(256), 0, nullptr, ds->ds, (unsigned long long)ds->n_texels, d);
+            e = hipGetLastError();
+        }
+        if (e == hipSuccess) e = hipMemcpy(&h, d, sizeof h, hipMemcpyDeviceToHost);
+        (void)hipFree(d);
+        if (e != hipSuccess) return rt_fail(RT_ERR_DEVICE, std::string("rt_device_selfcheck 4: ") + hipGetErrorString(e));
+        total += h;
+    }
+    *mismatches = total;
+    return RT_OK;
+#else
+    return rt_fail(RT_ERR_ARG, "rt_device_selfcheck 4: built without RT_SHADE_GATHER");
+#endif
+}
 }
 
 extern "C" {
 
 int rt_device_selfcheck(int32_t which, uint64_t *mismatches) {
     if (!mismatches) return rt_fail(RT_ERR_ARG, "rt_device_selfcheck: null output");
-    if (which < 0 || which > 3) return rt_fail(RT_ERR_ARG, "rt_device_selfcheck: unknown check " + std::to_string(which));
+    if (which < 0 || which > 4) return rt_fail(RT_ERR_ARG, "rt_device_selfcheck: unknown check " + std::to_string(which));
+    if (which == 4) return mat_selfcheck(mismatches);
     unsigned long long *d = nullptr;
     HIP_TRY(hipMalloc((void **)&d, sizeof *d));
     hipError_t e = hipMemset(d, 0, sizeof *d);
diff --git a/raytracing-hw_amd/csrc/rt_material.h b/raytracing-hw_amd/csrc/rt_material.h
--- /dev/null
+++ b/raytracing-hw_amd/csrc/rt_material.h
@@ -0,0 +1,55 @@
+#pragma once
+#include <cstddef>
+#include <cstdint>
+#include <cstring>
+#include <vector>
+
+namespace rtmat {
+
+constexpr int kRecDwords = 32;
+constexpr int kRecTex = 12;
+constexpr int kRecDesc = 16;
+
+inline void tile_textures(const std::vector<uint32_t> &info, const std::vector<uint8_t> &texels,
+                          std::vector<uint32_t> &info_out, std::vector<uint32_t> &out) {
+    const size_t n = info.size() / 4;
+    info_out = info;
+    out.clear();
+    for (size_t t = 0; t < n; ++t) {
+        const uint32_t off = info[4 * t], w = info[4 * t + 1], h = info[4 * t + 2];
+        const uint32_t tw = (w + 3) / 4, th = (h + 3) / 4;
+        const size_t base = out.size();
+        info_out[4 * t] = (uint32_t)base;
+        out.resize(base + (size_t)tw * th * 16, 0u);
+        for (uint32_t y = 0; y < h; ++y)
+            for (uint32_t x = 0; x < w; ++x) {
+                uint32_t v;
+                std::memcpy(&v, &texels[4 * ((size_t)off + (size_t)y * w + x)], 4);
+                out[base + ((size_t)(y >> 2) * tw + (x >> 2)) * 16 + (y & 3) * 4 + (x & 3)] = v;
+            }
+    }
+    if (out.empty()) out.resize(16, 0u);
+}
+
+inline bool build_records(const float *mesh_f, const int32_t *mesh_tex, size_t n_meshes, const uint32_t *tex_info,
+                          size_t n_textures, std::vector<uint32_t> &rec) {
+    rec.assign(n_meshes * kRecDwords, 0u);
+    for (size_t m = 0; m < n_meshes; ++m) {
+        uint32_t *r = &rec[m * kRecDwords];
+        std::memcpy(r, mesh_f + 12 * m, 12 * sizeof(float));
+        std::memcpy(r + kRecTex, mesh_tex + 4 * m, 4 * sizeof(int32_t));
+        for (int s = 0; s < 4; ++s) {
+            const int32_t t = mesh_tex[4 * m + s];
+            uint32_t *d = r + kRecDesc + 3 * s;
+            if (t < 0) {
+                d[0] = 0u; d[1] = 1u; d[2] = 1u;
+                continue;
+            }
+            if ((size_t)t >= n_textures) return false;
+            d[0] = tex_info[4 * (size_t)t]; d[1] = tex_info[4 * (size_t)t + 1]; d[2] = tex_info[4 * (size_t)t + 2];
+        }
+    }
+    return true;
+}
+
+}
diff --git a/raytracing-hw_amd/csrc/rt_mega.h b/raytracing-hw_amd/csrc/rt_mega.h
--- a/raytracing-hw_amd/csrc/rt_mega.h
+++ b/raytracing-hw_amd/csrc/rt_mega.h
@@ -317,7 +317,7 @@
                              float *out, const NodeRec &root, V3 color, LaneCtr c,
                              const unsigned long long *queue = nullptr);
 
-template <bool COUNT, bool FAST = false, bool CHAIN = false, class Stack, class ML>
+template <bool COUNT, bool FAST = false, bool CHAIN = false, int G = SHADE_TABLES, class Stack, class ML>
 __device__ __forceinline__ void mega_shade(ML &L, const DevScene &sc, const ShardGeom &g, const WfState &st,
                                            int spp, float *out, unsigned *cost, const NodeRec &root, Stack &stk,
                                            Counters &cnt, bool tail = false, bool park = false,
@@ -328,14 +328,29 @@
     bool next = false;
     const bool shaded = h.prim >= 0 && h.t < sc.max_distance;
     if (shaded) {
+        ShadeTri r1;
+        const ShadeTri *r1p = nullptr;
+#if RT_SHADE_GATHER && defined(__HIPCC__)
+        if constexpr (G != SHADE_TABLES) {
+            RT_CHECK(h.prim < sc.n_tris, 1, h.prim, h.prim = 0);
+            const float4 *tt = sc.tri + 3 * (size_t)h.prim, *ta = sc.tri_attr + 4 * (size_t)h.prim;
+            const float4 t0 = tt[0], t1 = tt[1];
+            r1 = ShadeTri{tt[2], ta[0], ta[1], ta[2], ta[3]};
+            r1p = &r1;
+            asm volatile("" ::"v"(t0.x), "v"(t1.x), "v"(r1.t2.x), "v"(r1.a0.x), "v"(r1.a1.x), "v"(r1.a2.x), "v"(r1.a3.x));
+            if constexpr (kUvRecompute) hit_uv_of(t0, t1, r1.t2, L.r, h);
+        } else
+#endif
+        {
 #if defined(__HIPCC__)
-        if constexpr (kUvRecompute) {
-            RT_CHECK(h.prim < sc.n_tris, 1, h.prim, h.prim = 0);
-            hit_uv(sc, L.r, h);
-        }
-#endif
+            if constexpr (kUvRecompute) {
+                RT_CHECK(h.prim < sc.n_tris, 1, h.prim, h.prim = 0);
+                hit_uv(sc, L.r, h);
+            }
+#endif
+        }
         Rng rng = lane_rng(L);
-        const bool cont = shade_hit<COUNT>(sc, L.r, h, rng, cnt, P, c.nv, stk);
+        const bool cont = shade_hit<COUNT, G>(sc, L.r, h, rng, cnt, P, c.nv, stk, r1p);
         lane_rng_set(L, rng);
         if (cont && c.power > 0) {
             c.power -= 1;
@@ -485,7 +500,8 @@
     mega_sample<COUNT, FAST>(L, sc, g, root, cnt);
 }
 
-template <bool COUNT, class Stack, class Nodes, bool FAST = false, bool LSPLIT = false, bool CHAIN = false, class ML>
+template <bool COUNT, class Stack, class Nodes, bool FAST = false, bool LSPLIT = false, bool CHAIN = false,
+          int G = SHADE_TABLES, class ML>
 __device__ __forceinline__ void mega_iterate(ML &L, bool shade_now, const DevScene &sc, const ShardGeom &g,
                                              const WfState &st, int spp, float *out, unsigned *cost,
                                              const NodeRec &root, Stack &stk, const Nodes &nodes, Counters &cnt,
@@ -504,7 +520,7 @@
     }
     if (shade_now) {
         if (L.state == M_READY)
-            mega_shade<COUNT, FAST, CHAIN>(L, sc, g, st, spp, out, cost, root, stk, cnt, tail, park, queue);
+            mega_shade<COUNT, FAST, CHAIN, G>(L, sc, g, st, spp, out, cost, root, stk, cnt, tail, park, queue);
     } else if (L.state == M_TRAV) {
         if (trav_step<COUNT>(sc, L.r, L.T, stk, nodes, cnt)) L.state = M_READY;
     }
diff --git a/raytracing-hw_amd/csrc/rt_path.h b/raytracing-hw_amd/csrc/rt_path.h
--- a/raytracing-hw_amd/csrc/rt_path.h
+++ b/raytracing-hw_amd/csrc/rt_path.h
@@ -88,6 +88,11 @@
     return lut[(srgb ? 0u : 256u) + byte];
 #endif
 }
+
+#ifndef RT_SHADE_GATHER
+#define RT_SHADE_GATHER 1
+#endif
+enum { SHADE_TABLES = 0, SHADE_GATHER_HOLD = 1 };
 
 struct DevScene {
     const float4 *tri;
@@ -111,6 +116,10 @@
     float cam_pos[3];
     float cam_axes[9];
     float tan_fov[2];
+#if RT_SHADE_GATHER
+    const uint4 *mat;
+    int any_nmap;
+#endif
 };
 
 struct Counters {
@@ -386,6 +395,56 @@
     return light_pdf<COUNT>(sc, point, direction, cnt, stk);
 }
 
+__device__ __forceinline__ int tex_f2i(float x) {
+#if defined(__HIP_DEVICE_COMPILE__)
+    return (int)x;
+#else
+    if (!(x == x)) return 0;
+    return x >= 2147483648.f ? 2147483647 : x < -2147483648.f ? (int)-2147483648LL : (int)x;
+#endif
+}
+#ifdef __HIPCC__
+constexpr bool kTexTiled = true;
+#else
+constexpr bool kTexTiled = false;
+#endif
+template <bool TILED = kTexTiled>
+__device__ __forceinline__ void tex_taps(uint32_t off, int W, int H, V2 p, uint32_t idx[4], float &dx, float &dy) {
+    p.x -= floorf(p.x);
+    p.y -= floorf(p.y);
+    p.x *= (float)W;
+    p.y *= (float)H;
+    const int px = tex_f2i(floorf(p.x)), py = tex_f2i(floorf(p.y));
+    dx = p.x - floorf(p.x);
+    dy = p.y - floorf(p.y);
+    auto wrap = [](int v, int n) {
+        v = v >= n ? v - n : v;
+        return v >= n ? v - n : v;
+    };
+#pragma unroll
+    for (int ddy = 0; ddy < 2; ++ddy)
+#pragma unroll
+        for (int ddx = 0; ddx < 2; ++ddx) {
+            const int x = wrap(px + ddx, W), y = wrap(py + ddy, H);
+            const uint32_t i = TILED ? (uint32_t)(((y >> 2) * ((W + 3) >> 2) + (x >> 2)) * 16 + (y & 3) * 4 + (x & 3))
+                                     : (uint32_t)(y * W + x);
+            idx[ddx * 2 + ddy] = off + i;
+        }
+}
+__device__ __forceinline__ V4 tex_decode(const float *lut, const uint32_t texel[4], float dx, float dy, bool srgb) {
+    float res[4];
+#pragma unroll
+    for (int c = 0; c < 4; ++c) {
+        float v[4];
+#pragma unroll
+        for (int k = 0; k < 4; ++k) {
+            const uint32_t byte = (texel[k] >> (8 * c)) & 0xffu;
+            v[k] = texel_decode(lut, byte, srgb);
+        }
+        res[c] = v[0] * (1 - dx) * (1 - dy) + v[1] * (1 - dx) * dy + v[2] * dx * (1 - dy) + v[3] * dx * dy;
+    }
+    return V4{res[0], res[1], res[2], res[3]};
+}
 __device__ __forceinline__ V4 tex_sample_ti(const DevScene &sc, const uint4 ti, V2 p, bool srgb) {
     const int W = (int)ti.y, H = (int)ti.z;
     p.x -= floorf(p.x);
@@ -724,54 +783,131 @@
     return c;
 }
 
+struct SlotTexels {
+    uint32_t x[4];
+    float dx, dy;
+};
 struct ShadeMid {
     V3 pos, N, dir;
     V2 tc;
     float r2, metallic;
     int mesh;
-};
-
-template <bool COUNT, class Rec>
+    int mt_b;
+    SlotTexels base;
+};
+
+struct ShadeTri {
+    float4 t2, a0, a1, a2, a3;
+};
+
+#if RT_SHADE_GATHER && defined(__HIPCC__)
+__device__ __forceinline__ SlotTexels slot_gather(const DevScene &sc, bool present, const uint32_t *d, V2 tc) {
+    SlotTexels o{{0u, 0u, 0u, 0u}, 0.f, 0.f};
+    if (__any(present)) {
+        uint32_t ix[4];
+        tex_taps(d[0], (int)d[1], (int)d[2], tc, ix, o.dx, o.dy);
+#pragma unroll
+        for (int k = 0; k < 4; ++k) o.x[k] = sc.texels[ix[k]];
+    }
+    return o;
+}
+#endif
+
+template <bool COUNT, int G = SHADE_TABLES, class Rec>
 __device__ __forceinline__ bool shade_pre(const DevScene &sc, const Ray &r, const Hit &hit, Rng &rng, Counters &cnt,
-                                          Rec &P, int &nv, ShadeMid &m) {
+                                          Rec &P, int &nv, ShadeMid &m, const ShadeTri *r1 = nullptr) {
     RT_PROF_BEGIN
     if (COUNT) cnt.hits++;
     int id = hit.prim;
     RT_CHECK(id >= 0 && id < sc.n_tris, 1, id, id = 0);
     RT_CHECK(nv >= 0 && nv < kMaxDepth - 1, 2, nv, nv = 0);
     const float u = hit.u, v = hit.v;
-    const float4 t2 = sc.tri[3 * id + 2];
+    const bool have_r1 = G != SHADE_TABLES && r1;
+    const float4 t2 = have_r1 ? r1->t2 : sc.tri[3 * id + 2];
     V3 ngeo{t2.y, t2.z, t2.w};
     bool inside = false;
     if (rtv::dot(r.d, ngeo) > 0) { inside = true; ngeo = rtv::neg(ngeo); }
-    const float4 a0 = sc.tri_attr[4 * id], a1 = sc.tri_attr[4 * id + 1], a2 = sc.tri_attr[4 * id + 2],
-                 a3 = sc.tri_attr[4 * id + 3];
+    const float4 a0 = have_r1 ? r1->a0 : sc.tri_attr[4 * id], a1 = have_r1 ? r1->a1 : sc.tri_attr[4 * id + 1],
+                 a2 = have_r1 ? r1->a2 : sc.tri_attr[4 * id + 2], a3 = have_r1 ? r1->a3 : sc.tri_attr[4 * id + 3];
     int mesh = __float_as_int(a3.w);
     RT_CHECK(mesh >= 0 && mesh < sc.n_meshes, 3, mesh, mesh = 0);
-    const float *mf = sc.mesh_f + 12 * mesh;
-    const int *mt = sc.mesh_tex + 4 * mesh;
-    const int mt_e = mt[3], mt_n = mt[1], mt_mr = mt[2];
-    const uint4 ti_e = sc.tex_info[mt_e >= 0 ? mt_e : 0], ti_n = sc.tex_info[mt_n >= 0 ? mt_n : 0],
-                ti_mr = sc.tex_info[mt_mr >= 0 ? mt_mr : 0];
+    float mrec[12];
+    const float *mf = mrec;
+    int mt_e, mt_n, mt_mr;
+    uint4 ti_e{}, ti_n{}, ti_mr{};
+    float4 g0{}, g1{}, g2{};
+    uint32_t dsc[12] = {};
+    SlotTexels se{}, sn{}, sm{};
+#if RT_SHADE_GATHER
+    if constexpr (G != SHADE_TABLES) {
+        const uint4 *rec = sc.mat + 8 * mesh;
+        const uint4 q0 = rec[0], q1 = rec[1], q2 = rec[2], q3 = rec[3], q4 = rec[4], q5 = rec[5], q6 = rec[6];
+        if (sc.any_nmap) {
+            g0 = sc.tri_tan[3 * id];
+            g1 = sc.tri_tan[3 * id + 1];
+            g2 = sc.tri_tan[3 * id + 2];
+        }
 #ifdef __HIPCC__
-    asm volatile("" ::"v"(ti_e.x), "v"(ti_n.x), "v"(ti_mr.x));
-#endif
+        asm volatile("" ::"v"(q0.x), "v"(q1.x), "v"(q2.x), "v"(q3.x), "v"(q4.x), "v"(q5.x), "v"(q6.x), "v"(g0.x), "v"(g1.x),
+                     "v"(g2.x));
+#endif
+        const uint32_t f[12] = {q0.x, q0.y, q0.z, q0.w, q1.x, q1.y, q1.z, q1.w, q2.x, q2.y, q2.z, q2.w};
+#pragma unroll
+        for (int k = 0; k < 12; ++k) mrec[k] = __uint_as_float(f[k]);
+        mt_n = (int)q3.y;
+        mt_mr = (int)q3.z;
+        mt_e = (int)q3.w;
+        const uint32_t d[12] = {q4.x, q4.y, q4.z, q4.w, q5.x, q5.y, q5.z, q5.w, q6.x, q6.y, q6.z, q6.w};
+#pragma unroll
+        for (int k = 0; k < 12; ++k) dsc[k] = d[k];
+        m.mt_b = (int)q3.x;
+    } else
+#endif
+    {
+        mf = sc.mesh_f + 12 * mesh;
+        const int *mt = sc.mesh_tex + 4 * mesh;
+        mt_e = mt[3], mt_n = mt[1], mt_mr = mt[2];
+        ti_e = sc.tex_info[mt_e >= 0 ? mt_e : 0], ti_n = sc.tex_info[mt_n >= 0 ? mt_n : 0],
+        ti_mr = sc.tex_info[mt_mr >= 0 ? mt_mr : 0];
+#ifdef __HIPCC__
+        asm volatile("" ::"v"(ti_e.x), "v"(ti_n.x), "v"(ti_mr.x));
+#endif
+    }
     const float w = 1 - u - v;
     const V2 tc{w * a2.y + u * a2.w + v * a3.y, w * a2.z + u * a3.x + v * a3.z};
+#if RT_SHADE_GATHER && defined(__HIPCC__)
+    if constexpr (G != SHADE_TABLES) {
+        se = slot_gather(sc, mt_e >= 0, dsc + 9, tc);
+        sn = slot_gather(sc, mt_n >= 0, dsc + 3, tc);
+        sm = slot_gather(sc, mt_mr >= 0, dsc + 6, tc);
+        m.base = slot_gather(sc, m.mt_b >= 0, dsc, tc);
+        asm volatile("" ::"v"(se.x[0]), "v"(se.x[1]), "v"(se.x[2]), "v"(se.x[3]), "v"(sn.x[0]), "v"(sn.x[1]), "v"(sn.x[2]),
+                     "v"(sn.x[3]), "v"(sm.x[0]), "v"(sm.x[1]), "v"(sm.x[2]), "v"(sm.x[3]), "v"(m.base.x[0]), "v"(m.base.x[1]),
+                     "v"(m.base.x[2]), "v"(m.base.x[3]));
+    }
+#endif
+    auto slot_sample = [&](const uint4 ti, const SlotTexels &t, bool srgb) {
+        if constexpr (G != SHADE_TABLES) return tex_decode(sc.lut, t.x, t.dx, t.dy, srgb);
+        else return tex_sample_ti(sc, ti, tc, srgb);
+    };
     V3 emission{mf[3], mf[4], mf[5]};
-    if (mt_e >= 0) emission = rtv::mulv(rtv::reduce(tex_sample_ti(sc, ti_e, tc, true)), emission);
+    if (mt_e >= 0) emission = rtv::mulv(rtv::reduce(slot_sample(ti_e, se, true)), emission);
     P.set_e(nv, emission);
     RT_PROF_SEG(0);
     V3 n0{a0.x, a0.y, a0.z}, n1{a0.w, a1.x, a1.y}, n2{a1.z, a1.w, a2.x};
     V3 lz = rtv::normal(rtv::add(rtv::add(rtv::mul(n0, w), rtv::mul(n1, u)), rtv::mul(n2, v)));
     V3 N = lz;
     if (mt_n >= 0) {
-        const float4 g0 = sc.tri_tan[3 * id], g1 = sc.tri_tan[3 * id + 1], g2 = sc.tri_tan[3 * id + 2];
+        if constexpr (G == SHADE_TABLES) {
+            g0 = sc.tri_tan[3 * id];
+            g1 = sc.tri_tan[3 * id + 1];
+            g2 = sc.tri_tan[3 * id + 2];
+        }
         V3 t0{g0.x, g0.y, g0.z}, t1{g1.x, g1.y, g1.z}, tt2{g2.x, g2.y, g2.z};
         V3 lx = rtv::normal(mul_vector_d(sc.mesh_nt + 16 * mesh,
                                          rtv::normal(rtv::add(rtv::add(rtv::mul(t0, w), rtv::mul(t1, u)), rtv::mul(tt2, v)))));
         V3 ly = rtv::mul(rtv::cross(lz, lx), g0.w);
-        V3 s = rtv::reduce(tex_sample_ti(sc, ti_n, tc, false));
+        V3 s = rtv::reduce(slot_sample(ti_n, sn, false));
         V3 ln = rtv::mul(rtv::addf(s, -0.5f), 2.f);
         N = rtv::normal(rtv::add(rtv::add(rtv::mul(lx, ln.x), rtv::mul(ly, ln.y)), rtv::mul(lz, ln.z)));
     }
@@ -779,7 +915,7 @@
     RT_PROF_SEG(1);
     float r2 = mf[7], metallic = mf[6];
     if (mt_mr >= 0) {
-        V4 mr = tex_sample_ti(sc, ti_mr, tc, false);
+        V4 mr = slot_sample(ti_mr, sm, false);
         float rr = mr.y * mr.y;
         r2 = rr * mf[7];
         metallic = mr.z * mf[6];
@@ -810,7 +946,7 @@
     return (cosine_pdf(N, dir) + lp + vndf_pdf(N, eye, r2, dir)) / 3;
 }
 
-template <class Rec>
+template <int G = SHADE_TABLES, class Rec>
 __device__ __forceinline__ bool shade_post(const DevScene &sc, const V3 rd, const ShadeMid &m, float pdf, Rec &P, int nv,
                                            Ray &r_out) {
     RT_PROF_BEGIN
@@ -818,15 +954,36 @@
     const V3 pos = m.pos, N = m.N, dir = m.dir, eye = rtv::neg(rd);
     const V2 tc = m.tc;
     const float r2 = m.r2, metallic = m.metallic;
-    const float *mf = sc.mesh_f + 12 * m.mesh;
-    const int *mt = sc.mesh_tex + 4 * m.mesh;
+    float mrec[9];
+    const float *mf = mrec;
+    const int *mt = nullptr;
+    int mt_b = -1;
+#if RT_SHADE_GATHER
+    if constexpr (G != SHADE_TABLES) {
+        const uint4 *rec = sc.mat + 8 * m.mesh;
+        const uint4 q0 = rec[0], q2 = rec[2];
+        mrec[0] = __uint_as_float(q0.x);
+        mrec[1] = __uint_as_float(q0.y);
+        mrec[2] = __uint_as_float(q0.z);
+        mrec[8] = __uint_as_float(q2.x);
+        mt_b = m.mt_b;
+    } else
+#endif
+    {
+        mf = sc.mesh_f + 12 * m.mesh;
+        mt = sc.mesh_tex + 4 * m.mesh;
+    }
     const float coeff = 1 / pdf;
     const V3 half = rtv::normal(rtv::sub(dir, rd));
     const float vis = smith(r2, N, eye, dir) * (1.f / (4 * fabsf(rtv::dot(N, rd)) * fabsf(rtv::dot(N, dir))));
     const float spec = ggx(r2, N, half) * vis;
     const float VdotH = fabsf(rtv::dot(eye, half));
     V3 base{mf[0], mf[1], mf[2]};
-    if (mt[0] >= 0) base = rtv::mulv(rtv::reduce(tex_sample(sc, mt[0], tc, true)), base);
+    if constexpr (G == SHADE_TABLES) {
+        if (mt[0] >= 0) base = rtv::mulv(rtv::reduce(tex_sample(sc, mt[0], tc, true)), base);
+    } else if (mt_b >= 0) {
+        base = rtv::mulv(rtv::reduce(tex_decode(sc.lut, m.base.x, m.base.dx, m.base.dy, true)), base);
+    }
     const float p5 = rtm::pow5_glibc(1.f - VdotH);
     const V3 fres{base.x + (1.f - base.x) * p5, base.y + (1.f - base.y) * p5, base.z + (1.f - base.z) * p5};
     const V3 metal = rtv::mul(fres, spec);
@@ -841,15 +998,15 @@
 }
 
 
-template <bool COUNT, class Rec, class Stack>
+template <bool COUNT, int G = SHADE_TABLES, class Rec, class Stack>
 __device__ bool shade_hit(const DevScene &sc, Ray &r, const Hit &hit, Rng &rng, Counters &cnt, Rec &P, int &nv,
-                          Stack &stk) {
+                          Stack &stk, const ShadeTri *r1 = nullptr) {
     ShadeMid m;
-    if (!shade_pre<COUNT>(sc, r, hit, rng, cnt, P, nv, m)) return false;
+    if (!shade_pre<COUNT, G>(sc, r, hit, rng, cnt, P, nv, m, r1)) return false;
     RT_PROF_BEGIN
     const float pdf = scene_pdf<COUNT>(sc, m.pos, m.N, rtv::neg(r.d), m.r2, m.dir, cnt, stk);
     RT_PROF_SEG(4);
-    return shade_post(sc, r.d, m, pdf, P, nv, r);
+    return shade_post<G>(sc, r.d, m, pdf, P, nv, r);
 }
 template <bool COUNT, class Rec>
 __device__ bool shade_hit(const DevScene &sc, Ray &r, const Hit &hit, Rng &rng, Counters &cnt, Rec &P, int &nv) {
diff --git a/raytracing-hw_amd/csrc/rt_wavefront.h b/raytracing-hw_amd/csrc/rt_wavefront.h
--- a/raytracing-hw_amd/csrc/rt_wavefront.h
+++ b/raytracing-hw_amd/csrc/rt_wavefront.h
@@ -511,6 +511,12 @@
 #endif
 constexpr bool kUvRecompute = RT_UV_RECOMPUTE != 0;
 
+__device__ __forceinline__ void hit_uv_of(const float4 t0, const float4 t1, const float4 t2, const Ray &r, Hit &h) {
+    TriHit th;
+    tri_hit_bl(V3{t0.x, t0.y, t0.z}, V3{t0.w, t1.x, t1.y}, V3{t1.z, t1.w, t2.x}, r, th);
+    h.u = th.u;
+    h.v = th.v;
+}
 __device__ __forceinline__ void hit_uv(const DevScene &sc, const Ray &r, Hit &h) {
     const float4 *t = sc.tri + 3 * (size_t)h.prim;
     const float4 t0 = t[0], t1 = t[1], t2 = t[2];
```

Measured after the change: 2109, median of 6. 2.4% higher.
